# RManLuo/MAMDR

Hardware: AMD Instinct MI355X
Metric: domain-steps/sec (higher is better)
Workload: dtype f32; 1 GPU; mlp_meta_mamdr Taobao-10 bs=1024 (frozen pretrained tables); global_batch=1024, domains=10, step_definition=one MAMDR meta-epoch (DN + DR phases, all outer updates), parallelism=single GPU

## Files before the change

include/mamdr_hip.h:

```cpp
#ifndef MAMDR_HIP_H
#define MAMDR_HIP_H

#include <stddef.h>
#include <stdint.h>

#ifdef __cplusplus
extern "C" {
#endif

#define MAMDR_ABI_VERSION 19

enum {
    MAMDR_OK = 0,
    MAMDR_EINVAL = -1,
    MAMDR_ESTATE = -2,
    MAMDR_EHIP = -3,
    MAMDR_ENOTBUILT = -4
};

enum { MAMDR_TOWER_MLP = 0, MAMDR_TOWER_DEEPFM = 1, MAMDR_TOWER_STAR = 2,
       MAMDR_TOWER_WDL = 3,
       MAMDR_TOWER_PNN = 4,
       MAMDR_TOWER_NFM = 5 };
enum { MAMDR_SPLIT_TRAIN = 0, MAMDR_SPLIT_VAL = 1, MAMDR_SPLIT_TEST = 2 };
// ... 30 lines not shown
    int32_t n_item;
    int32_t n_domain;
    int32_t emb_dim;
    int32_t hidden[3];
    int32_t max_batch;
    int32_t emb_trainable;
    float dropout;
    float l2_emb;
    float l2_linear;
    float adam_beta1, adam_beta2, adam_eps;
    int32_t uncertainty_weight;
} mamdr_config;

const char* mamdr_last_error(void);
int mamdr_abi_version(void);
const char* mamdr_env_switches(void);
int mamdr_env_unknown(void);

int mamdr_create(const mamdr_config* cfg, void* stream, mamdr_ctx** out);
int mamdr_destroy(mamdr_ctx* ctx);

int64_t mamdr_param_count(const mamdr_ctx* ctx);
int64_t mamdr_meta_count(const mamdr_ctx* ctx);
int64_t mamdr_aux_count(const mamdr_ctx* ctx);
int mamdr_bind_aux(mamdr_ctx* ctx, float* d_aux);
int mamdr_param_segment(const mamdr_ctx* ctx, int seg, int64_t* offset, int64_t* count);

int mamdr_bind_state(mamdr_ctx* ctx, float* d_params, float* d_adam_m, float* d_adam_v);
int mamdr_optimizer_reset(mamdr_ctx* ctx);
int mamdr_bind_accumulator(mamdr_ctx* ctx, float* d_acc);
int64_t mamdr_optimizer_steps(const mamdr_ctx* ctx);
int mamdr_set_counters(mamdr_ctx* ctx, int64_t optimizer_steps, int64_t dropout_steps);
int mamdr_sync_tables(mamdr_ctx* ctx);
int64_t mamdr_table_flushes(const mamdr_ctx* ctx, int32_t forced_only);

int mamdr_bind_table(mamdr_ctx* ctx, int seg, const float* d_rows, int64_t n_rows);

int mamdr_bind_domain_data(mamdr_ctx* ctx, int domain, int split, const int32_t* d_uid,
                           const int32_t* d_pid, const int32_t* d_domain, const float* d_label,
                           int64_t n_rows);

int mamdr_train_steps(mamdr_ctx* ctx, int domain, const int32_t* d_perm, int64_t first_step,
                      int64_t n_steps, int32_t batch, uint32_t dropout_seed, int32_t optimizer,
                      float lr, float* d_loss_out);
int mamdr_train_steps_n(mamdr_ctx* ctx, int domain, const int32_t* d_perm, int64_t pass_rows, int64_t first_step,
                        int64_t n_steps, int32_t batch, uint32_t dropout_seed, int32_t optimizer, float lr,
                        float* d_loss_out);

int mamdr_eval_domain(mamdr_ctx* ctx, int domain, int split, int32_t batch, float* d_loss_out,
                      uint32_t* d_hist, float* d_pred_out);

int mamdr_gather_rows(mamdr_ctx* ctx, int domain, int split, const int32_t* d_perm,
                      int64_t first_row, int64_t n_rows, float* d_out);

int mamdr_interp(float* d_dst, const float* d_a, const float* d_b, float scale, int64_t n,
                 void* stream);
int mamdr_moving_average(float* d_unbiased, float* d_biased, const float* d_value, float decay, float denom,
                         int64_t n, void* stream);
int mamdr_merge(float* d_dst, const float* d_theta, const float* d_phi, int32_t mode, int64_t n,
                void* stream);
int mamdr_dr_advance(float* d_phi, float* d_w, float* d_merged, const float* d_theta, float gamma, int32_t mode,
                     int32_t assign_model, int64_t n, void* stream);
int mamdr_dr_advance_live(mamdr_ctx* ctx, float* d_phi, float* d_merged, const float* d_theta, float gamma, int32_t mode,
                          int32_t assign_model, int64_t meta_off, int64_t n);
int mamdr_sub(float* d_dst, const float* d_a, const float* d_b, int64_t n, void* stream);
int mamdr_accumulate(float* d_acc, const float* d_a, const float* d_b, const float* d_shared,
                     float divisor, int64_t n, void* stream);
int mamdr_apply_accumulated(float* d_dst, float* d_acc, float divisor, float scale, int64_t n,
                            void* stream);
int mamdr_adam_apply(float* d_p, float* d_m, float* d_v, const float* d_g, float grad_scale, float lr,
                     float beta1, float beta2, float eps, float beta1_power, float beta2_power, int64_t n,
                     void* stream);
int mamdr_copy(float* d_dst, const float* d_src, int64_t n, void* stream);
int mamdr_pcgrad_project(float* d_final, float* d_aux, const int64_t* h_offsets, const int64_t* h_rows,
                         const int32_t* h_cols, int32_t n_seg, void* stream);

int mamdr_shuffle_perm(int64_t n, int64_t buffer_size, uint64_t seed, int32_t* h_out);
int mamdr_shuffle_perms(int32_t n_passes, const int64_t* h_n, int64_t buffer_size, const uint64_t* h_seeds,
                        int32_t* h_out);

int mamdr_profile_enable(mamdr_ctx* ctx, int32_t enable);
int mamdr_pregather_passes(mamdr_ctx* ctx, int32_t n_passes, const int32_t* h_domains, const int32_t* const* h_d_perms,
                           const int64_t* h_pass_rows, int32_t batch);
int64_t mamdr_pregather_hits(const mamdr_ctx* ctx);
int64_t mamdr_pregather_launches(const mamdr_ctx* ctx);
int mamdr_step_path(const mamdr_ctx* ctx, int32_t batch);
int mamdr_set_tower_tile(mamdr_ctx* ctx, int32_t rows);
int mamdr_tower_tile(const mamdr_ctx* ctx, int32_t batch);
int64_t mamdr_dropout_steps(const mamdr_ctx* ctx);
int mamdr_profile_reset(mamdr_ctx* ctx);
int mamdr_profile_read(mamdr_ctx* ctx, int32_t kernel, double* total_ms, int64_t* launches);

enum { MAMDR_GRAPH_SHARED_BOTTOM = 0,
       MAMDR_GRAPH_MMOE = 1,
       MAMDR_GRAPH_PLE = 2,
       MAMDR_GRAPH_NFM = 3,
       MAMDR_GRAPH_PNN = 4,
       MAMDR_GRAPH_CCPM = 5,
       MAMDR_GRAPH_AUTOINT = 6,
       MAMDR_GRAPH_MLP = 7,
       MAMDR_GRAPH_WDL = 8,
       MAMDR_GRAPH_DEEPFM = 9,
       MAMDR_GRAPH_STAR = 10 };
typedef struct mamdr_graph mamdr_graph;
typedef struct mamdr_graph_config {
    int32_t abi_version;
    int32_t kind;
    int32_t n_user, n_item, n_domain, emb_dim, max_batch, emb_trainable;
    int32_t n_expert_hidden; int32_t expert_hidden[4];
    int32_t n_tower_hidden;  int32_t tower_hidden[4];
    int32_t n_gate_hidden;   int32_t gate_hidden[4];
    int32_t num_experts;
    int32_t shared_expert_num, specific_expert_num;
    float dropout, l2_emb, adam_beta1, adam_beta2, adam_eps;
    float l2_linear;
    int32_t uncertainty_weight;
    int32_t star_norm;
    int32_t star_dense;
    int32_t auxiliary_dim;
} mamdr_graph_config;
const char* mamdr_graph_last_error(void);
int mamdr_graph_create(const mamdr_graph_config* cfg, void* stream, mamdr_graph** out);
int mamdr_graph_destroy(mamdr_graph* g);
int64_t mamdr_graph_param_count(const mamdr_graph* g);
int32_t mamdr_graph_tensor_count(const mamdr_graph* g);
int mamdr_graph_tensor_info(const mamdr_graph* g, int32_t i, char* name, int32_t name_cap, int64_t* offset, int64_t* rows,
                            int64_t* cols);
int mamdr_graph_task_ranges(const mamdr_graph* g, int domain, int64_t* shared_off, int64_t* shared_count, int64_t* task_off,
                            int64_t* task_count);
int mamdr_graph_bind_state(mamdr_graph* g, float* d_params, float* d_adam_m, float* d_adam_v);
int mamdr_graph_optimizer_reset(mamdr_graph* g);
int mamdr_graph_set_adam_eps(mamdr_graph* g, float eps);
int64_t mamdr_graph_optimizer_steps(const mamdr_graph* g);
int64_t mamdr_graph_aux_count(const mamdr_graph* g);
int mamdr_graph_bind_aux(mamdr_graph* g, float* d_aux);
int64_t mamdr_graph_launch_count(void);
int64_t mamdr_graph_dropout_steps(const mamdr_graph* g);
int mamdr_graph_set_counters(mamdr_graph* g, int64_t optimizer_steps, int64_t dropout_steps);
int mamdr_graph_bind_table(mamdr_graph* g, int seg, const float* d_rows, int64_t n_rows);
int mamdr_graph_bind_domain_data(mamdr_graph* g, int domain, int split, const int32_t* d_uid, const int32_t* d_pid,
                                 const int32_t* d_domain, const float* d_label, int64_t n_rows);
int mamdr_graph_train_steps(mamdr_graph* g, int domain, const int32_t* d_perm, int64_t first_step, int64_t n_steps,
                            int32_t batch, uint32_t dropout_seed, int32_t optimizer, float lr, float* d_loss_out);
int mamdr_graph_train_steps_n(mamdr_graph* g, int domain, const int32_t* d_perm, int64_t pass_rows, int64_t first_step,
                              int64_t n_steps, int32_t batch, uint32_t dropout_seed, int32_t optimizer, float lr,
                              float* d_loss_out);
int mamdr_graph_bind_accumulator(mamdr_graph* g, float* d_acc);
int mamdr_graph_eval_domain(mamdr_graph* g, int domain, int split, int32_t batch, float* d_loss_out, uint32_t* d_hist,
                            float* d_pred_out);

#ifdef __cplusplus
}
#endif
#endif
```

mamdr_amd/_lib.py:

```python
import ctypes as C
import os

HERE = os.path.dirname(os.path.abspath(__file__))
LIB_PATH = os.environ.get("MAMDR_LIB_PATH") or os.path.join(HERE, "libmamdr_hip.so")

ABI_VERSION = 19
OK, EINVAL, ESTATE, EHIP, ENOTBUILT = 0, -1, -2, -3, -4
TOWER_MLP, TOWER_DEEPFM, TOWER_STAR, TOWER_WDL, TOWER_PNN, TOWER_NFM = 0, 1, 2, 3, 4, 5
SPLIT_TRAIN, SPLIT_VAL, SPLIT_TEST = 0, 1, 2
OPT_ADAM, OPT_SGD, OPT_ACCUMULATE = 0, 1, 2
MERGE_PLUS, MERGE_TIMES = 0, 1
(SEG_USER_EMB, SEG_ITEM_EMB, SEG_DOMAIN_EMB, SEG_W0, SEG_W1, SEG_W2, SEG_B0, SEG_B1, SEG_B2, SEG_WO,
 SEG_GB, SEG_LIN_USER, SEG_LIN_ITEM, SEG_LIN_DOMAIN) = range(14)
SEG_NAMES = ("user_emb", "item_emb", "domain_emb", "W0", "W1", "W2", "b0", "b1", "b2", "wo", "gb",
             "lin_user", "lin_item", "lin_domain",
             "Ws0", "Ws1", "Ws2", "bs0", "bs1", "bs2", "pn_gamma_shared", "pn_beta_shared", "pn_gamma_spec",
             "pn_beta_spec", "Wd0", "Wd1", "Wd2", "bd0", "bd1", "bd2",
             "log_var",
             "W0x")
KERNEL_FWD_BWD, KERNEL_WGRAD, KERNEL_UPDATE, KERNEL_EVAL, KERNEL_GATHER, KERNEL_EMB_SWEEP, KERNEL_AUX, KERNEL_FLUSH = range(8)
KERNEL_NAMES = ("k_tower<train>", "k_wgrad", "k_update", "k_tower<eval>", "k_gather", "k_emb_sweep",
                "other launches of a step (include/mamdr_hip.h: MAMDR_KERNEL_AUX)", "k_emb_flush")


class MamdrError(RuntimeError):
    def __init__(self, code, text):
        RuntimeError.__init__(self, "libmamdr_hip error %d: %s" % (code, text))
        self.code = code


class NotBuiltError(MamdrError, NotImplementedError):
    pass


class Config(C.Structure):
    _fields_ = [
        ("abi_version", C.c_int32), ("tower", C.c_int32), ("n_user", C.c_int32), ("n_item", C.c_int32),
        ("n_domain", C.c_int32), ("emb_dim", C.c_int32), ("hidden", C.c_int32 * 3), ("max_batch", C.c_int32),
        ("emb_trainable", C.c_int32), ("dropout", C.c_float), ("l2_emb", C.c_float), ("l2_linear", C.c_float),
        ("adam_beta1", C.c_float), ("adam_beta2", C.c_float), ("adam_eps", C.c_float),
        ("uncertainty_weight", C.c_int32),
    ]


GRAPH_SHARED_BOTTOM, GRAPH_MMOE, GRAPH_PLE, GRAPH_NFM, GRAPH_PNN, GRAPH_CCPM, GRAPH_AUTOINT = 0, 1, 2, 3, 4, 5, 6
GRAPH_MLP, GRAPH_WDL, GRAPH_DEEPFM = 7, 8, 9
GRAPH_STAR = 10
STAR_NORMS = {"none": 0, "pn": 1, "bn": 2}
STAR_DENSES = {"dense": 0, "star": 1}


class GraphConfig(C.Structure):
    _fields_ = [
        ("abi_version", C.c_int32), ("kind", C.c_int32), ("n_user", C.c_int32), ("n_item", C.c_int32),
        ("n_domain", C.c_int32), ("emb_dim", C.c_int32), ("max_batch", C.c_int32), ("emb_trainable", C.c_int32),
        ("n_expert_hidden", C.c_int32), ("expert_hidden", C.c_int32 * 4),
        ("n_tower_hidden", C.c_int32), ("tower_hidden", C.c_int32 * 4),
        ("n_gate_hidden", C.c_int32), ("gate_hidden", C.c_int32 * 4),
        ("num_experts", C.c_int32), ("shared_expert_num", C.c_int32), ("specific_expert_num", C.c_int32),
        ("dropout", C.c_float), ("l2_emb", C.c_float), ("adam_beta1", C.c_float), ("adam_beta2", C.c_float),
        ("adam_eps", C.c_float), ("l2_linear", C.c_float), ("uncertainty_weight", C.c_int32),
        ("star_norm", C.c_int32), ("star_dense", C.c_int32), ("auxiliary_dim", C.c_int32),
    ]


_VP, _I32, _I64, _U32, _U64, _F = C.c_void_p, C.c_int32, C.c_int64, C.c_uint32, C.c_uint64, C.c_float

SIGNATURES = {
    "mamdr_last_error": (C.c_char_p, []),
    "mamdr_abi_version": (C.c_int, []),
    "mamdr_env_switches": (C.c_char_p, []),
    "mamdr_env_unknown": (C.c_int, []),
    "mamdr_create": (C.c_int, [C.POINTER(Config), _VP, C.POINTER(_VP)]),
    "mamdr_destroy": (C.c_int, [_VP]),
    "mamdr_param_count": (_I64, [_VP]),
    "mamdr_param_segment": (C.c_int, [_VP, C.c_int, C.POINTER(_I64), C.POINTER(_I64)]),
    "mamdr_meta_count": (_I64, [_VP]),
    "mamdr_aux_count": (_I64, [_VP]),
    "mamdr_bind_aux": (C.c_int, [_VP, _VP]),
    "mamdr_bind_state": (C.c_int, [_VP, _VP, _VP, _VP]),
    "mamdr_optimizer_reset": (C.c_int, [_VP]),
    "mamdr_optimizer_steps": (_I64, [_VP]),
    "mamdr_set_counters": (C.c_int, [_VP, _I64, _I64]),
    "mamdr_table_flushes": (_I64, [_VP, _I32]),
    "mamdr_pregather_passes": (_I32, [_VP, _I32, _VP, _VP, _VP, _I32]),
    "mamdr_pregather_hits": (_I64, [_VP]),
    "mamdr_pregather_launches": (_I64, [_VP]),
    "mamdr_sync_tables": (C.c_int, [_VP]),
    "mamdr_bind_accumulator": (C.c_int, [_VP, _VP]),
    "mamdr_bind_table": (C.c_int, [_VP, C.c_int, _VP, _I64]),
    "mamdr_bind_domain_data": (C.c_int, [_VP, C.c_int, C.c_int, _VP, _VP, _VP, _VP, _I64]),
    "mamdr_train_steps": (C.c_int, [_VP, C.c_int, _VP, _I64, _I64, _I32, _U32, _I32, _F, _VP]),
    "mamdr_train_steps_n": (C.c_int, [_VP, C.c_int, _VP, _I64, _I64, _I64, _I32, _U32, _I32, _F, _VP]),
    "mamdr_eval_domain": (C.c_int, [_VP, C.c_int, C.c_int, _I32, _VP, _VP, _VP]),
    "mamdr_gather_rows": (C.c_int, [_VP, C.c_int, C.c_int, _VP, _I64, _I64, _VP]),
    "mamdr_interp": (C.c_int, [_VP, _VP, _VP, _F, _I64, _VP]),
    "mamdr_moving_average": (C.c_int, [_VP, _VP, _VP, _F, _F, _I64, _VP]),
    "mamdr_merge": (C.c_int, [_VP, _VP, _VP, _I32, _I64, _VP]),
    "mamdr_dr_advance": (C.c_int, [_VP, _VP, _VP, _VP, _F, _I32, _I32, _I64, _VP]),
    "mamdr_dr_advance_live": (C.c_int, [_VP, _VP, _VP, _VP, _F, _I32, _I32, _I64, _I64]),
    "mamdr_sub": (C.c_int, [_VP, _VP, _VP, _I64, _VP]),
    "mamdr_accumulate": (C.c_int, [_VP, _VP, _VP, _VP, _F, _I64, _VP]),
    "mamdr_apply_accumulated": (C.c_int, [_VP, _VP, _F, _F, _I64, _VP]),
    "mamdr_adam_apply": (C.c_int, [_VP, _VP, _VP, _VP, _F, _F, _F, _F, _F, _F, _F, _I64, _VP]),
    "mamdr_copy": (C.c_int, [_VP, _VP, _I64, _VP]),
    "mamdr_pcgrad_project": (C.c_int, [_VP, _VP, _VP, _VP, _VP, _I32, _VP]),
    "mamdr_shuffle_perm": (C.c_int, [_I64, _I64, _U64, _VP]),
    "mamdr_shuffle_perms": (C.c_int, [_I32, _VP, _I64, _VP, _VP]),
    "mamdr_step_path": (C.c_int, [_VP, _I32]),
    "mamdr_dropout_steps": (_I64, [_VP]),
    "mamdr_set_tower_tile": (C.c_int, [_VP, _I32]),
    "mamdr_tower_tile": (C.c_int, [_VP, _I32]),
    "mamdr_profile_enable": (C.c_int, [_VP, _I32]),
    "mamdr_profile_reset": (C.c_int, [_VP]),
    "mamdr_profile_read": (C.c_int, [_VP, _I32, C.POINTER(C.c_double), C.POINTER(_I64)]),
    "mamdr_graph_last_error": (C.c_char_p, []),
    "mamdr_graph_create": (C.c_int, [C.POINTER(GraphConfig), _VP, C.POINTER(_VP)]),
    "mamdr_graph_destroy": (C.c_int, [_VP]),
    "mamdr_graph_param_count": (_I64, [_VP]),
    "mamdr_graph_tensor_count": (_I32, [_VP]),
    "mamdr_graph_tensor_info": (C.c_int, [_VP, _I32, C.c_char_p, _I32, C.POINTER(_I64), C.POINTER(_I64), C.POINTER(_I64)]),
    "mamdr_graph_task_ranges": (C.c_int, [_VP, C.c_int, C.POINTER(_I64), C.POINTER(_I64), C.POINTER(_I64), C.POINTER(_I64)]),
    "mamdr_graph_bind_state": (C.c_int, [_VP, _VP, _VP, _VP]),
    "mamdr_graph_optimizer_reset": (C.c_int, [_VP]),
    "mamdr_graph_set_adam_eps": (C.c_int, [_VP, _F]),
    "mamdr_graph_aux_count": (_I64, [_VP]),
    "mamdr_graph_bind_aux": (C.c_int, [_VP, _VP]),
    "mamdr_graph_launch_count": (_I64, []),
    "mamdr_graph_optimizer_steps": (_I64, [_VP]),
    "mamdr_graph_dropout_steps": (_I64, [_VP]),
    "mamdr_graph_set_counters": (C.c_int, [_VP, _I64, _I64]),
    "mamdr_graph_bind_table": (C.c_int, [_VP, C.c_int, _VP, _I64]),
    "mamdr_graph_bind_domain_data": (C.c_int, [_VP, C.c_int, C.c_int, _VP, _VP, _VP, _VP, _I64]),
    "mamdr_graph_train_steps": (C.c_int, [_VP, C.c_int, _VP, _I64, _I64, _I32, _U32, _I32, _F, _VP]),
    "mamdr_graph_train_steps_n": (C.c_int, [_VP, C.c_int, _VP, _I64, _I64, _I64, _I32, _U32, _I32, _F, _VP]),
    "mamdr_graph_bind_accumulator": (C.c_int, [_VP, _VP]),
    "mamdr_graph_eval_domain": (C.c_int, [_VP, C.c_int, C.c_int, _I32, _VP, _VP, _VP]),
}

_lib = None


def load():
    global _lib
    if _lib is not None:
        return _lib
    import torch
    if not os.path.exists(LIB_PATH):
        raise ImportError("%s not found: run `python -c 'import __graft_entry__ as g; g.build()'` "
                          "(there is no CPU fallback for the MAMDR hot path)" % LIB_PATH)
    lib = C.CDLL(LIB_PATH)
    for name, (res, args) in SIGNATURES.items():
        fn = getattr(lib, name)
        fn.restype = res
        fn.argtypes = args
    if lib.mamdr_abi_version() != ABI_VERSION:
        raise ImportError("libmamdr_hip.so ABI %d != binding ABI %d" % (lib.mamdr_abi_version(), ABI_VERSION))
    lib.mamdr_env_unknown()
    _lib = lib
    return lib


def env_switches():
    rows = load().mamdr_env_switches().decode("utf-8").strip().split("\n")
    return [tuple(r.split("\t")) for r in rows]


def check(code, graph=False):
    if code != OK:
        text = (load().mamdr_graph_last_error() if graph else load().mamdr_last_error()).decode("utf-8", "replace")
# ... 5 lines not shown
```

mamdr_amd/csrc/env_registry.h:

```cpp
#pragma once

namespace mamdr {

struct EnvSwitch {
    const char* name;
    const char* reader;
    const char* effect;
};

static const EnvSwitch kEnvSwitches[] = {
    {"MAMDR_DENSE_ADAM", "lib,bench", "1: per-step dense sweep of trainable tables instead of the lazy replay (same bits)"},
    {"MAMDR_LAZY_FLUSH_EVERY", "lib", "steps between forced replays of lagging table rows (default 32)"},
    {"MAMDR_LAZY_LOG_CAP", "lib", "capacity of the alpha ring of the lazy table Adam (tests: force it to wrap)"},
    {"MAMDR_NO_TAILFUSE", "lib", "1: the table kernels as launches of their own instead of riders"},
    {"MAMDR_TOWER_TILE", "lib,bench", "rows per tower workgroup: 0 automatic, 4, 16 (initial value of mamdr_set_tower_tile)"},
    {"MAMDR_FUSED", "lib", "0: slab path everywhere; 2: k_wgrad_adam path for every batch size (default: up to 4 rows x CUs)"},
    {"MAMDR_DM_EACH", "lib", "1: k_dm_finish after every step (diagnostic; same bits)"},
    {"MAMDR_DM_CALL", "lib", "1: k_dm_finish closes every call (diagnostic; same bits)"},
    {"MAMDR_T4_NO_W1L", "lib", "1: k_tower4 without the W1 image in LDS (diagnostic)"},
    {"MAMDR_NO_W2_DIRECT", "lib", "1: k_transpose_w opens a call instead of the W2-in-place tower instance"},
    {"MAMDR_NO_PREGATHER", "lib,bench", "1: no k_pass_prep; the tower gathers its rows itself"},
    {"MAMDR_STAR_DENSE_SLICES", "lib", "1: every per-domain Star slice swept every step (diagnostic; same bits)"},
    {"MAMDR_GRAPH_NO_DEFER", "lib", "1: a pair of weight-gradient launches per layer instead of the queued flat grid"},
    {"MAMDR_GRAPH_TILE32_BELOW", "lib", "row count below which the 32 x 32 GEMM tile is used (0: 64 x 64 everywhere)"},
    {"MAMDR_GRAPH_NO_TAIL_OPT", "lib", "1: k_graph_adam as a launch of its own (same bits)"},
    {"MAMDR_LIB_PATH", "host,bench", "load this build of the library instead of mamdr_amd/libmamdr_hip.so (tools/build_variant.sh)"},
    {"MAMDR_LANES", "host", "lanes per process (overrides train.lanes)"},
    {"MAMDR_SHARE_GPU", "host", "1: every rank of run.py on device 0 over gloo (testing on a 1-GPU box)"},
    {"MAMDR_COMM_TIMEOUT", "host", "seconds: process-group timeout of run.py"},
    {"MAMDR_TAIL_SYNC", "host", "sum: tensors outside theta / phi combined by sum instead of the step-weighted mean"},
    {"MAMDR_NO_PASS_WINDOW", "host", "1: every call gathers its own pass (no k_pass_prep_multi windows)"},
    {"MAMDR_PASS_WINDOW_ROWS", "host", "row budget of a pass window"},
    {"MAMDR_PNN_ENGINE", "host", "graph: PNN on the generic-layer engine (default: step kernels)"},
    {"MAMDR_NFM_ENGINE", "host", "graph: NFM on the generic-layer engine"},
    {"MAMDR_STAR_ENGINE", "host", "graph: Star's PartitionedNorm + StarFCN form on the generic-layer engine (default: step kernels)"},
    {"MAMDR_BENCH_*", "bench", "bench.py knobs: _BATCH _ROW_SCALE _DN_MODE _NO_PREFETCH _PREP_TIMING _PREWARM_S _SHARE_GPU _COMM_TIMEOUT _SKIP_<WORKLOAD>"},
    {"MAMDR_DIAG_FLAGS", "tools", "extra -D flags of the stamp tools' diagnostic builds"},
    {"MAMDR_STAMPS_PREBUILT", "tools", "stamp tools: use an already built variant"},
    {"MAMDR_DIST_AUC_SCALE", "tools", "row scale of tools/dist_auc.py"},
    {"MAMDR_TEST_*", "tests", "test-suite knobs: _ALL_CPUS _BLAS_THREADS _NO_ORACLE_POOL _NO_PINNING _REPORT_FRAC"},
};
constexpr int kNumEnvSwitches = (int)(sizeof(kEnvSwitches) / sizeof(kEnvSwitches[0]));

}
```

mamdr_amd/csrc/fused_kernels.hip:

```cpp
#include <hip/hip_ext.h>

#include "mamdr_kernels.h"

namespace mamdr {

constexpr int FZ_THREADS = 512;
constexpr int FZ_WAVES = 8;
constexpr int FZ_RING = 32;
constexpr int FZ_SBLK = DM_PARTS;
constexpr int FZ_SC = 8;
constexpr int FZ_OUTB = 2;
constexpr int FZ_T0 = (2 * EMB / 16) * (H1 / 32);
constexpr int FZ_T1 = (H1 / 16) * (H2 / 32);
constexpr int FZ_T2 = (H2 / 16) * (H3 / 32);
constexpr int FZ_TILES = FZ_T0 + FZ_T1 + FZ_T2;

#define FZSTAMP(k) MAMDR_STAMP(MAMDR_CYCLES, a.stamps && threadIdx.x == 0, a.stamps[blockIdx.x * 8 + (k)])
#define FZREAL(k) MAMDR_STAMP(MAMDR_REALTIME, a.stamps && threadIdx.x == 0, a.stamps[blockIdx.x * 8 + (k)])

__device__ __forceinline__ void fz_store(const FusedArgs& a, int e, float p, float m, float v) {
    if (a.optimizer == 2) {
        a.m[e] = m;
        return;
    }
    if (a.optimizer == 0) {
        a.m[e] = m;
        a.v[e] = v;
    }
    a.p[e] = p;
}

__device__ __forceinline__ void fz_share(int n_slots, int w, int& s0, int& s1) {
    const int per = (n_slots + FZ_WAVES - 1) / FZ_WAVES;
    s0 = min(w * per, n_slots);
    s1 = min(s0 + per, n_slots);
}

template <bool CSUM>
__device__ __forceinline__ void fz_dense(const float* __restrict__ A, int lda, const float* __restrict__ B, int ldb,
                                         int s0, int s1, f32x4 (&acc)[2], f32x2& csum) {
    const int lane = threadIdx.x & 63, j = lane & 15, kq = lane >> 4;
    const int n = s1 - s0;
    if (n <= 0) return;
    const unsigned aoff = (unsigned)(kq * lda + j), boff = (unsigned)(kq * ldb + 2 * j);
    const float* arow = A + (size_t)(4 * s0) * lda;
    const float* brow = B + (size_t)(4 * s0) * ldb;
    const size_t astep = (size_t)4 * lda, bstep = (size_t)4 * ldb;
    const int last = n - 1;
    float ra[FZ_RING];
    f32x2 rb[FZ_RING];
#pragma unroll
    for (int u = 0; u < FZ_RING; ++u) {
        const int idx = min(u, last);
        ra[u] = (arow + idx * astep)[aoff];
        rb[u] = *reinterpret_cast<const f32x2*>(brow + idx * bstep + boff);
    }
    __builtin_amdgcn_sched_barrier(0);
    const int passes = (n + FZ_RING - 1) / FZ_RING;
    int base = 0;
    for (int pass = 0; pass + 1 < passes; ++pass, base += FZ_RING) {
#pragma unroll
        for (int u = 0; u < FZ_RING; ++u) {
            acc[0] = MAMDR_MFMA16(ra[u], rb[u][0], acc[0]);
            acc[1] = MAMDR_MFMA16(ra[u], rb[u][1], acc[1]);
            if (CSUM) csum += rb[u];
            const int idx = min(base + u + FZ_RING, last);
            ra[u] = (arow + idx * astep)[aoff];
            rb[u] = *reinterpret_cast<const f32x2*>(brow + idx * bstep + boff);
            __builtin_amdgcn_sched_barrier(0);
        }
    }
#pragma unroll
    for (int u = 0; u < FZ_RING; ++u) {
        const float keep = (base + u < n) ? 1.0f : 0.0f;
        const f32x2 b2 = rb[u] * keep;
        acc[0] = MAMDR_MFMA16(ra[u], b2[0], acc[0]);
        acc[1] = MAMDR_MFMA16(ra[u], b2[1], acc[1]);
        if (CSUM) csum += b2;
        __builtin_amdgcn_sched_barrier(0);
    }
}

template <int MT>
__device__ __forceinline__ void fz_onehot(const int32_t* __restrict__ domrow, const float* __restrict__ B, int ldb,
                                          int s0, int s1, f32x4 (&acc)[4]) {
    const int lane = threadIdx.x & 63, j = lane & 15, kq = lane >> 4;
    const int n = s1 - s0;
    if (n <= 0) return;
    const unsigned boff = (unsigned)(kq * ldb + (j & (FZ_SC - 1)));
    const int32_t* drow = domrow + 4 * s0;
    const float* brow = B + (size_t)(4 * s0) * ldb;
    const size_t bstep = (size_t)4 * ldb;
    const int last = n - 1;
    int rd[FZ_RING];
    float rb[FZ_RING];
#pragma unroll
    for (int u = 0; u < FZ_RING; ++u) {
        const int idx = min(u, last);
// ... 278 lines not shown
            rd[u] = (drow + idx * 4)[(unsigned)kq];
        }
        __builtin_amdgcn_sched_barrier(0);
        const int passes = (n + FZ_RING - 1) / FZ_RING;
        int base = 0;
        for (int pass = 0; pass + 1 < passes; ++pass, base += FZ_RING) {
#pragma unroll
            for (int u = 0; u < FZ_RING; ++u) {
                const float bv = j == 0 ? rd[u] : 0.f;
                acc[0] = MAMDR_MFMA16(ra[u][0], bv, acc[0]);
                acc[1] = MAMDR_MFMA16(ra[u][1], bv, acc[1]);
                sg += bv;
                const int idx = min(base + u + FZ_RING, last);
                ra[u] = *reinterpret_cast<const f32x2*>(arow + (size_t)idx * 4 * ACT_LD + aoff);
                rd[u] = (drow + idx * 4)[(unsigned)kq];
                __builtin_amdgcn_sched_barrier(0);
            }
        }
#pragma unroll
        for (int u = 0; u < FZ_RING; ++u) {
            const float bv = (j == 0 && base + u < n) ? rd[u] : 0.f;
            acc[0] = MAMDR_MFMA16(ra[u][0], bv, acc[0]);
            acc[1] = MAMDR_MFMA16(ra[u][1], bv, acc[1]);
            sg += bv;
            __builtin_amdgcn_sched_barrier(0);
        }
    }
    if (j == 0) {
#pragma unroll
        for (int r = 0; r < 4; ++r)
            *reinterpret_cast<f32x2*>(lds + w * 32 + 2 * (4 * kq + r)) = (f32x2){acc[0][r], acc[1][r]};
    }
    sg += __shfl_xor(sg, 16);
    sg += __shfl_xor(sg, 32);
    if (lane == 0) lds[256 + w] = sg;
    FZSTAMP(2);
    __syncthreads();
    FZSTAMP(3);
    if (tid < 32) {
        float g = lds[tid];
#pragma unroll
        for (int ww = 1; ww < FZ_WAVES; ++ww) g += lds[ww * 32 + tid];
        const int e = a.L.wo + 32 * ob + tid;
        float p = a.p[e], m = a.optimizer == 1 ? 0.f : a.m[e], v = a.optimizer == 0 ? a.v[e] : 0.f;
        opt_step(a, g, p, m, v);
        fz_store(a, e, p, m, v);
    } else if (tid == 64 && ob == 0) {
        float g = lds[256];
#pragma unroll
        for (int ww = 1; ww < FZ_WAVES; ++ww) g += lds[256 + ww];
        const int e = a.L.gb;
        float p = a.p[e], m = a.optimizer == 1 ? 0.f : a.m[e], v = a.optimizer == 0 ? a.v[e] : 0.f;
        opt_step(a, g, p, m, v);
        fz_store(a, e, p, m, v);
    }
    FZSTAMP(4);
}

__device__ __forceinline__ void fz_loss_body(const FusedArgs& a, float* lds) {
    const int tid = threadIdx.x;
    float ss = 0.f, ls = 0.f;
    for (int e = tid; e < a.n_domain * EMB; e += FZ_THREADS) ss = fmaf(a.p[e], a.p[e], ss);
    for (int e = tid; e < a.n_loss_tiles; e += FZ_THREADS) ls += a.loss_part[e];
    for (int o = 32; o > 0; o >>= 1) {
        ss += __shfl_xor(ss, o);
        ls += __shfl_xor(ls, o);
    }
    if ((tid & 63) == 0) {
        lds[tid >> 6] = ss;
        lds[8 + (tid >> 6)] = ls;
    }
    __syncthreads();
    if (tid == 0) {
        float sst = 0.f, lst = 0.f;
        for (int ww = 0; ww < FZ_WAVES; ++ww) {
            sst += lds[ww];
            lst += lds[8 + ww];
        }
        const float reg = a.l2_emb * a.frozen_sumsq[0] + a.l2_emb * a.frozen_sumsq[1] + a.l2_emb * sst;
        a.loss_out[0] = lst / (float)a.rows + reg;
    }
}

__global__ __launch_bounds__(FZ_THREADS) void k_wgrad_adam(const FusedArgs a) {
    extern __shared__ __attribute__((aligned(16))) float lds[];
    const int b = (int)blockIdx.x;
    FZSTAMP(0);
    FZREAL(5);
    if (b < FZ_SBLK) fz_s_body(a, b, lds);
    else if (b < FZ_SBLK + FZ_TILES) fz_tile_body(a, b - FZ_SBLK, lds);
    else if (b < FZ_SBLK + FZ_TILES + FZ_OUTB) fz_out_body(a, b - FZ_SBLK - FZ_TILES, lds);
    else fz_loss_body(a, lds);
    FZREAL(6);
}

void launch_wgrad_adam(const FusedArgs& a, hipStream_t s) {
    const int grid = FZ_SBLK + FZ_TILES + FZ_OUTB + (a.loss_out ? 1 : 0);
    const size_t lds = (size_t)fz_lds_floats(a.n_domain) * sizeof(float);
    if (lds > 65536) {
        static const bool big_lds_set = hipFuncSetAttribute(reinterpret_cast<const void*>(k_wgrad_adam),
                                                            hipFuncAttributeMaxDynamicSharedMemorySize,
                                                            (int)(fz_lds_floats(64) * sizeof(float))) == hipSuccess;
        (void)big_lds_set;
    }
    MAMDR_LAUNCH(k_wgrad_adam, dim3(grid), dim3(FZ_THREADS), lds, s, a);
}

__global__ __launch_bounds__(256) void k_dm_finish(const DmStep q, float* live_p, float* live_m, float* live_v) {
    const int i = blockIdx.x * 256 + threadIdx.x;
    if (i >= q.n_domain * (EMB / 4)) return;
    const int d = i / (EMB / 4), c4 = i - d * (EMB / 4);
    f32x4 p, m, v;
    dm_step4(q, d, c4, p, m, v);
    const size_t row = (size_t)d * EMB + 4 * c4;
    if (q.optimizer != 2) *reinterpret_cast<f32x4*>(live_p + row) = p;
    if (q.optimizer != 1) *reinterpret_cast<f32x4*>(live_m + row) = m;
    if (q.optimizer == 0) *reinterpret_cast<f32x4*>(live_v + row) = v;
}

void launch_dm_finish(const DmStep& q, float* live_p, float* live_m, float* live_v, hipStream_t s) {
    MAMDR_LAUNCH(k_dm_finish, dim3((q.n_domain * (EMB / 4) + 255) / 256), dim3(256), 0, s, q, live_p, live_m, live_v);
}

template <typename P>
__device__ __forceinline__ void pass_prep_row(const P& a, const float* user_tab, const float* item_tab, int n_user, int n_item,
                                              int n_domain, int64_t pos0, float* xpre, int32_t* pdom, float* plabel, int64_t i) {
    const int lane = threadIdx.x & 63;
    if (i >= a.n) {
        if (i < a.n + 16) {
            *reinterpret_cast<f32x4*>(xpre + (size_t)i * (2 * EMB) + 4 * lane) = (f32x4){0.f, 0.f, 0.f, 0.f};
            if (lane == 0) {
                pdom[i] = a.pad_dom;
                plabel[i] = 0.f;
            }
        }
        return;
    }
    int64_t src = a.perm ? (int64_t)a.perm[pos0 + i] : pos0 + i;
    src = src < 0 ? 0 : (src >= a.n_rows_split ? a.n_rows_split - 1 : src);
    int u = a.uid[src], it = a.pid[src];
    u = u < 0 ? 0 : (u >= n_user ? n_user - 1 : u);
    it = it < 0 ? 0 : (it >= n_item ? n_item - 1 : it);
    const float* row = lane < 32 ? user_tab + (size_t)u * EMB + 4 * lane : item_tab + (size_t)it * EMB + 4 * (lane - 32);
    const f32x4 v = *reinterpret_cast<const f32x4*>(row);
    __builtin_nontemporal_store(v, reinterpret_cast<f32x4*>(xpre + (size_t)i * (2 * EMB) + 4 * lane));
    if (lane == 0) {
        int d = a.dom[src];
        pdom[i] = d < 0 ? 0 : (d >= n_domain ? n_domain - 1 : d);
        plabel[i] = a.label[src];
    }
}
__global__ __launch_bounds__(256) void k_pass_prep(const PassPrepArgs a) {
    if ((int)blockIdx.x >= a.n_prep_wgs) {
        transpose_w_elem(a.tw_dense, a.tw_L, a.tw_wT, ((int)blockIdx.x - a.n_prep_wgs) * 256 + (int)threadIdx.x);
        return;
    }
    pass_prep_row(a, a.user_tab, a.item_tab, a.n_user, a.n_item, a.n_domain, a.pos0, a.xpre, a.pdom, a.plabel,
                  (int64_t)blockIdx.x * 4 + (threadIdx.x >> 6));
}
__global__ __launch_bounds__(256) void k_pass_prep_multi(const PassPrepMultiArgs a) {
    int k = 0;
    while (k + 1 < a.n_pass && (int)blockIdx.x >= a.wg_end[k]) ++k;
    const int wg0 = k ? a.wg_end[k - 1] : 0;
    const PassPrepMultiArgs::Pass& p = a.p[k];
    pass_prep_row(p, a.user_tab, a.item_tab, a.n_user, a.n_item, a.n_domain, (int64_t)0, a.xpre + (size_t)p.out_off * (2 * EMB),
                  a.pdom + p.out_off, a.plabel + p.out_off, (int64_t)((int)blockIdx.x - wg0) * 4 + (threadIdx.x >> 6));
}
void launch_pass_prep_multi(const PassPrepMultiArgs& a, hipStream_t s) {
    if (a.n_pass <= 0) return;
    MAMDR_LAUNCH(k_pass_prep_multi, dim3((unsigned)a.wg_end[a.n_pass - 1]), dim3(256), 0, s, a);
}
void launch_pass_prep(const PassPrepArgs& a0, hipStream_t s) {
    if (a0.n <= 0) return;
    PassPrepArgs a = a0;
    a.n_prep_wgs = (int)((a.n + 16 + 3) / 4);
    MAMDR_LAUNCH(k_pass_prep, dim3((unsigned)(a.n_prep_wgs + (a.tw_wT ? TRANSPOSE_WGS : 0))), dim3(256), 0, s, a);
}

}
```

mamdr_amd/csrc/mamdr_api.hip:

```cpp
#include <hip/hip_runtime.h>

#include <cmath>
#include <cstdarg>
#include <cstdio>
#include <cstdlib>
#include <cstring>
#include <new>
#include <string>
#include <utility>
#include <vector>

#include "../../include/mamdr_hip.h"
#include "mamdr_kernels.h"
#include "env_registry.h"

using namespace mamdr;

namespace mamdr {
thread_local hipEvent_t g_prof_stop = nullptr;
}

namespace {

thread_local char g_err[512] = "";
// ... 4 lines not shown
    vsnprintf(g_err, sizeof(g_err), fmt, ap);
    va_end(ap);
    return code;
}

#define HIP_TRY(expr)                                                                          \
    do {                                                                                       \
        hipError_t e_ = (expr);                                                                \
        if (e_ != hipSuccess) return fail(MAMDR_EHIP, "%s: %s", #expr, hipGetErrorString(e_)); \
    } while (0)

struct SplitData {
    const int32_t* uid = nullptr;
    const int32_t* pid = nullptr;
    const int32_t* dom = nullptr;
    const float* label = nullptr;
    int64_t n = 0;
    bool bound = false;
};

struct EventPair {
    hipEvent_t a, b;
    bool own_a = true;
};

}

struct mamdr_ctx {
    mamdr_config cfg;
    hipStream_t stream = nullptr;
    DenseLayout L;
    int64_t table_floats = 0;
    bool deepfm = false;
    bool nfm = false;
    bool pnn = false;
    float* ipbuf = nullptr;
    bool star = false;
    StarLayout SL;
    StarAuxLayout AL;
    int64_t n_meta = 0;
    float* aux = nullptr;
    float* eff = nullptr;
    float* pn = nullptr;
    float* star_part = nullptr;
    float* star_sums = nullptr;
    float* star_dmpart = nullptr;
    int64_t lin_user_off = 0;
    int64_t lin_item_off = 0;
    int64_t n_params = 0;
    float* params = nullptr;
    float* adam_m = nullptr;
    float* adam_v = nullptr;
    float* accum = nullptr;
    const float* user_tab = nullptr;
    const float* item_tab = nullptr;
    std::vector<SplitData> data;
    int64_t adam_t = 0;
    float b1p = 1.0f, b2p = 1.0f;
    uint32_t global_step = 0;
    int rows_pad_max = 0;
    float* acts = nullptr;
    float* dz = nullptr;
    float* dlogit = nullptr;
    float* w0dom_copy = nullptr;
    float* dm_copy = nullptr;
    bool lin_w0dom = false;
    float* wT = nullptr;
    bool fused = false;
    float* star_alpha = nullptr;
    int star_dense_slices = 0;
    int t4_no_w1l = 0;
    int fused_max_batch = 1024;
    int tower4_max_rows = 2048;
    float* pdm = nullptr;
    float* xpre = nullptr;
    int32_t* pdom = nullptr;
    float* plabel = nullptr;
    int64_t pre_cap = 0;
    struct PgEntry { int domain; const int32_t* perm; int64_t n, off; int batch; };
    std::vector<PgEntry> pg;
    size_t pg_pos = 0;
    int64_t pg_hits = 0;
    int64_t pg_launches = 0;
    bool use_pre = true;
    float* dmsnap[2] = {nullptr, nullptr};
    int dm_cur = 0;
    DmStep dm_pending{};
    bool dm_finish_call = false;
    bool wT_valid = false;
    bool w1t_unread = false;
    bool w2_direct_ok = true;
    bool dm_finish_each = false;
    int tower_tile = 0;
    float* dxe = nullptr;
    int32_t* urow = nullptr;
    int32_t* irow = nullptr;
    int32_t* map_u = nullptr;
    int32_t* map_i = nullptr;
    float* gbuf_u = nullptr;
    float* gbuf_i = nullptr;
    int32_t* hasdup_u = nullptr;
    int32_t* hasdup_i = nullptr;
    bool lazy = false;
    bool tables_dirty = false;
    int32_t* last_u = nullptr;
    int32_t* last_i = nullptr;
    float* alpha_log = nullptr;
    int log_cap = 1 << 16;
    int flush_every = 32;
    int64_t flush_t = 0;
    int64_t n_flush = 0;
    int64_t n_flush_forced = 0;
    float* fmq = nullptr;
    float* glin_u = nullptr;
    float* glin_i = nullptr;
    int32_t* domrow = nullptr;
    float* loss_part = nullptr;
    float* eval_part = nullptr;
    int64_t eval_part_cap = 0;
    float* slabs = nullptr;
    bool tail_fuse = true;
    int32_t* urow_alt = nullptr;
    int32_t* irow_alt = nullptr;
    int32_t* map_u_alt = nullptr;
    int32_t* map_i_alt = nullptr;
    bool rows_ready = false;
    bool catchup_ready = false;
    int slab_ld = 0;
    int s2_off = 0;
    TileDesc* tiles = nullptr;
    int n_tiles = 0;
    float* thresholds = nullptr;
    float* frozen_sumsq = nullptr;
    float* sumsq_partials = nullptr;
#ifdef MAMDR_STAMPS
    unsigned long long* stamps = nullptr;
#endif
    bool profile = false;
    std::vector<hipEvent_t> ev_pool;
    void ev_pool_push(hipEvent_t e) { ev_pool.push_back(e); }
    hipEvent_t prev_b = nullptr;
    bool chain_ok = false;
    std::vector<EventPair> ev[MAMDR_KERNEL_COUNT];
};

namespace {

std::vector<TileDesc> build_tiles(const DenseLayout& L, int n_domain, bool deepfm, int s2_off, bool lin_w0dom, bool star,
                                  bool pnn = false, bool nfm = false) {
    std::vector<TileDesc> t;
    struct G { int a_off, M, b_off, N, dst; };
    const G gemms[3] = {{0, XDIM, 0, H1, L.w0}, {XDIM, H1, H1, H2, L.w1}, {XDIM + H1, H2, H1 + H2, H3, L.w2}};
    for (const G& g : gemms)
        for (int m0 = (nfm && g.dst == L.w0) ? 2 * EMB : 0; m0 < ((lin_w0dom && g.dst == L.w0) ? 2 * EMB : g.M); m0 += 64)
            for (int n0 = 0; n0 < g.N; n0 += 64)
                t.push_back(TileDesc{0, g.a_off + m0, 0, g.b_off + n0, g.dst + m0 * g.N + n0, g.N, 64, 64, 1});
    const int boff[3] = {L.b0, L.b1, L.b2}, bn[3] = {H1, H2, H3}, zoff[3] = {0, H1, H1 + H2};
    for (int l = 0; l < 3; ++l)
        for (int n0 = 0; n0 < bn[l]; n0 += 32) t.push_back(TileDesc{1, 0, 0, zoff[l] + n0, boff[l] + n0, 0, 1, 32});
    for (int m0 = 0; m0 < H3; m0 += 32) t.push_back(TileDesc{0, XDIM + H1 + H2 + m0, 1, 0, L.wo + m0, 1, 32, 1});
    t.push_back(TileDesc{1, 0, 1, 0, L.gb, 0, 1, 1});
    for (int m0 = 0; m0 < (star ? 0 : n_domain); m0 += 32)
        for (int n0 = 0; n0 < H1; n0 += 32) {
            const int mv = n_domain - m0 < 32 ? n_domain - m0 : 32;
            t.push_back(TileDesc{2, m0, 0, n0, L.alloc + m0 * H1 + n0, H1, mv, 32});
        }
// ... 169 lines not shown
    }
    c->tables_dirty = false;
    c->flush_t = c->adam_t;
    c->n_flush += 1;
}

static void fill_rows_args(const mamdr_ctx* c, const SplitData& d, const int32_t* d_perm, int64_t row_base, int rows,
                           int rows_pad, float alpha, int64_t t, bool alt, EmbRowsArgs& ra) {
    memset(&ra, 0, sizeof(ra));
    ra.uid = d.uid;
    ra.pid = d.pid;
    ra.perm = d_perm;
    ra.row_base = row_base;
    ra.n_rows_split = d.n;
    ra.rows = rows;
    ra.rows_pad = rows_pad;
    ra.n_user = c->cfg.n_user;
    ra.n_item = c->cfg.n_item;
    ra.urow = alt ? c->urow_alt : c->urow;
    ra.irow = alt ? c->irow_alt : c->irow;
    ra.map_u = alt ? c->map_u_alt : c->map_u;
    ra.map_i = alt ? c->map_i_alt : c->map_i;
    ra.alpha_log = c->alpha_log;
    ra.log_idx = (int)(t & (c->log_cap - 1));
    ra.alpha = alpha;
}

static void emb_pre_step(mamdr_ctx* c, const SplitData& d, const int32_t* d_perm, int64_t row_base, int rows,
                         int rows_pad, float alpha, float omb1, float omb2) {
    if (c->adam_t - c->flush_t >= c->log_cap - 2 || c->adam_t - c->flush_t > c->flush_every) {
        c->adam_t -= 1;
        if (c->tables_dirty) c->n_flush_forced += 1;
        sync_tables(c);
        c->adam_t += 1;
    }
    if (!c->rows_ready) {
        EmbRowsArgs ra;
        fill_rows_args(c, d, d_perm, row_base, rows, rows_pad, alpha, c->adam_t, false, ra);
        Prof p(c, MAMDR_KERNEL_AUX);
        launch_emb_rows(ra, c->stream);
    }
    c->rows_ready = false;
    if (!c->catchup_ready) {
        EmbStepArgs ea;
        fill_emb_args(c, MAMDR_OPT_ADAM, alpha, omb1, omb2, table_two_l2(c), rows, c->star ? XDIM : 2 * EMB, ea);
        Prof p(c, MAMDR_KERNEL_AUX);
        launch_emb_catchup(ea, c->stream);
    }
    c->catchup_ready = false;
    c->tables_dirty = true;
}

static void emb_post_step(mamdr_ctx* c, int32_t optimizer, float alpha, float omb1, float omb2, int rows) {
    EmbStepArgs ea;
    fill_emb_args(c, optimizer, alpha, omb1, omb2, table_two_l2(c), rows, c->star ? XDIM : 2 * EMB, ea);
    if (c->lazy && optimizer == MAMDR_OPT_ADAM) {
        ea.flags_done = 1;
        ea.apply_now = 1;
        {
            Prof p(c, MAMDR_KERNEL_EMB_SWEEP);
            launch_emb_reduce(ea, c->stream);
        }
        if (c->deepfm) {
            Prof p(c, MAMDR_KERNEL_AUX);
            launch_lin_sweep(ea, c->stream);
        }
        return;
    }
    launch_emb_reduce(ea, c->stream);
    prof_break(c);
    {
        Prof p(c, MAMDR_KERNEL_EMB_SWEEP);
        launch_emb_sweep(ea, c->stream);
    }
    if (c->deepfm) {
        Prof p(c, MAMDR_KERNEL_AUX);
        launch_lin_sweep(ea, c->stream);
    }
}

static int64_t pad_rows(int64_t rows) { return (rows + TILE_ROWS - 1) / TILE_ROWS * TILE_ROWS; }
static int rows_at(int64_t pass_rows, int64_t row_base, int batch) { return (int)std::min<int64_t>(batch, pass_rows - row_base); }
static bool takes_fused_path(const mamdr_ctx* c, int64_t batch) { return c->fused && pad_rows(batch) <= c->fused_max_batch; }
static bool takes_tower4(const mamdr_ctx* c, int64_t rows_pad) {
    return !c->star && c->tower_tile != 16 && (c->tower_tile == 4 || rows_pad <= c->tower4_max_rows);
}
static bool w1t_unread_now(const mamdr_ctx* c) {
    if (!c->fused || c->tower_tile == 16) return false;
    const int64_t max4 = c->tower_tile == 4 ? c->rows_pad_max : std::min<int64_t>(c->tower4_max_rows, c->rows_pad_max);
    return tower4_never_streams(max4, c->t4_no_w1l);
}
static int wgrad_groups(int rows_pad, int* rpg) {
    int r = rows_pad <= 512 ? 256 : (rows_pad <= 1024 ? 128 : (rows_pad <= 4096 ? 256 : 512));
    int groups = (rows_pad + r - 1) / r;
    if (groups > WGRAD_MAX_GROUPS) {
        r = ((rows_pad + WGRAD_MAX_GROUPS - 1) / WGRAD_MAX_GROUPS + 7) / 8 * 8;
        groups = (rows_pad + r - 1) / r;
    }
    *rpg = r;
    return groups;
}
static float adam_alpha(float lr, float b1p, float b2p) { return lr * sqrtf(1.0f - b2p) / (1.0f - b1p); }
static float advance_step(mamdr_ctx* c, int32_t optimizer, float lr) {
    if (optimizer != MAMDR_OPT_ADAM) return lr;
    c->adam_t += 1;
    c->b1p = c->b1p * c->cfg.adam_beta1;
    c->b2p = c->b2p * c->cfg.adam_beta2;
    return adam_alpha(lr, c->b1p, c->b2p);
}

enum class StepPath { star, fused, slab };
struct CallPlan {
    const SplitData* d;
    int domain;
    const int32_t* perm;
    int64_t pass_rows, first_step, n_steps;
    int batch;
    int32_t optimizer;
    float lr, omb1, omb2;
    float* loss_out;
    uint32_t seed, drop_thresh;
    float keep_scale;
    int use_dropout;
    StepPath path = StepPath::slab;
    bool tail = false;
    bool pre = false;
    bool pre_cached = false;
    int64_t pre_pos0 = 0, pre_n = 0, pre_base = 0;
    bool need_wT = false;
    bool build_wT = false;
    bool w2_direct = false;
    bool star_lazy = false;
};

static void plan_call(mamdr_ctx* c, CallPlan& P) {
    P.path = c->star ? StepPath::star : (takes_fused_path(c, P.batch) ? StepPath::fused : StepPath::slab);
    const bool fused = P.path == StepPath::fused;
    const bool accumulate = P.optimizer == MAMDR_OPT_ACCUMULATE;
    P.tail = c->tail_fuse && c->cfg.emb_trainable && c->lazy && P.optimizer == MAMDR_OPT_ADAM && !c->profile && !P.loss_out;
    const int first_rows = rows_at(P.pass_rows, P.first_step * P.batch, P.batch);
    P.need_wT = takes_tower4(c, pad_rows(rows_at(P.pass_rows, (P.first_step + P.n_steps - 1) * P.batch, P.batch)));
    P.pre_pos0 = P.first_step * P.batch;
    P.pre_n = std::min<int64_t>((P.first_step + P.n_steps) * P.batch, P.pass_rows) - P.pre_pos0;
    P.pre = fused && c->use_pre && P.pre_n > 0;
    P.build_wT = P.need_wT && !c->wT_valid;
    if (P.build_wT && P.pre && c->w2_direct_ok && !accumulate && !c->t4_no_w1l && c->tower_tile != 16 && tower4_w1l_ready() &&
        tower4_takes_w1l(first_rows, c->t4_no_w1l)) {
        P.build_wT = false;
        P.w2_direct = true;
    }
    if (P.build_wT && !accumulate && !fused && !c->star && !takes_tower4(c, pad_rows(first_rows)) && P.n_steps > 1)
        P.build_wT = false;
    if (P.pre) {
        for (size_t k = c->pg_pos; k < c->pg.size(); ++k) {
            const mamdr_ctx::PgEntry& e = c->pg[k];
            if (e.domain == P.domain && e.perm == P.perm && e.n == P.pass_rows && e.batch == P.batch) {
                c->pg_pos = k;
                P.pre_base = e.off + P.pre_pos0;
                P.pre_cached = true;
                c->pg_hits += 1;
                break;
            }
        }
        if (!P.pre_cached) c->pg.clear();
    }
    P.star_lazy = c->star && P.optimizer == MAMDR_OPT_ADAM && P.n_steps >= 2 && !P.loss_out && !c->star_dense_slices &&
                  c->cfg.n_domain > 1;
}

static void fill_next_step(const mamdr_ctx* c, const CallPlan& P, int64_t row_base, EmbRowsArgs& nr, EmbStepArgs& nea) {
    const int rows = rows_at(P.pass_rows, row_base, P.batch);
    const float alpha = adam_alpha(P.lr, c->b1p * c->cfg.adam_beta1, c->b2p * c->cfg.adam_beta2);
    fill_rows_args(c, *P.d, P.perm, row_base, rows, (int)pad_rows(rows), alpha, c->adam_t + 1, true, nr);
    fill_emb_args(c, MAMDR_OPT_ADAM, alpha, P.omb1, P.omb2, table_two_l2(c), rows, c->star ? XDIM : 2 * EMB, nea);
    nea.t_now = (int)c->adam_t + 1;
    nea.t[0].brow = c->urow_alt;
    nea.t[0].map = c->map_u_alt;
    nea.t[1].brow = c->irow_alt;
    nea.t[1].map = c->map_i_alt;
}

static void take_next_rows(mamdr_ctx* c) {
    std::swap(c->urow, c->urow_alt);
    std::swap(c->irow, c->irow_alt);
    std::swap(c->map_u, c->map_u_alt);
    std::swap(c->map_i, c->map_i_alt);
    c->rows_ready = true;
    c->catchup_ready = true;
    c->tables_dirty = true;
}

static int star_step(mamdr_ctx* c, const CallPlan& P, int64_t s, float alpha) {
    const SplitData& d = *P.d;
    const int domain = P.domain;
    const int32_t optimizer = P.optimizer;
    const float omb1 = P.omb1, omb2 = P.omb2;
    float* const loss_out = P.loss_out ? P.loss_out + s : nullptr;
    const int64_t row_base = (P.first_step + s) * P.batch;
    const int rows = rows_at(P.pass_rows, row_base, P.batch);
    const int rows_pad = (int)pad_rows(rows);
    const int chunks = (rows + STAR_CHUNK - 1) / STAR_CHUNK;
    const int lazy_idx = (int)(s & (STAR_ALPHA_CAP - 1));
    const bool next = P.tail && s + 1 < P.n_steps;
    EmbRowsArgs nr;
    EmbStepArgs nea;
    if (next) fill_next_step(c, P, row_base + P.batch, nr, nea);
    float* blk = c->params + c->table_floats;
    TowerArgs ta;
    fill_tower_common(c, d, ta);
    ta.perm = P.perm;
    ta.row_base = row_base;
    ta.rows = rows;
    ta.batch = rows;
    if (c->cfg.emb_trainable && c->lazy && optimizer == MAMDR_OPT_ADAM)
        emb_pre_step(c, d, P.perm, row_base, rows, rows_pad, alpha, omb1, omb2);
    StarPrepArgs pa;
    memset(&pa, 0, sizeof(pa));
    pa.blk = blk;
    pa.SL = c->SL;
    pa.L = c->L;
    pa.n_domain = c->cfg.n_domain;
    pa.d = domain;
    pa.eff = c->eff;
    pa.pn = c->pn;
    pa.part = c->star_part;
    pa.n_chunks = chunks;
    pa.rows = rows;
    pa.aux = c->aux;
    pa.AL = c->AL;
    pa.train = 1;
    pa.skip_eff = P.star_lazy && s > 0 ? 1 : 0;
    {
        Prof p(c, MAMDR_KERNEL_AUX);
        launch_star_stats(ta, c->star_part, c->aux + c->AL.steps + domain, c->stream);
        launch_star_prep(pa, c->stream);
    }

    ta.dense = c->eff;
    ta.pn_aff = c->pn;
    ta.pn_part = c->star_part;
    ta.use_dropout = 0;
    ta.keep_scale = 1.0f;
    ta.acts = c->acts;
    ta.dz = c->dz;
    ta.dlogit = c->dlogit;
    ta.domrow = c->domrow;
    ta.dxe = c->dxe;
// ... 101 lines not shown
    ua.opt.eps = c->cfg.adam_eps;
    ua.opt.two_l2 = 0.f;
    if (P.star_lazy) {
        ua.only_live = 1;
        ua.alpha_log = c->star_alpha;
        ua.log_idx = lazy_idx;
        if (s + 1 < P.n_steps) ua.eff_out = c->eff;
    }
    {
        Prof p(c, MAMDR_KERNEL_UPDATE);
        ua.dm_elsewhere = no_apply ? 1 : 0;
        if (next) launch_star_update_catchup(ua, nea, no_apply ? &ba : nullptr, c->stream);
        else launch_star_update(ua, c->stream);
    }
    if (next) take_next_rows(c);
    if (c->cfg.emb_trainable && !P.tail) emb_post_step(c, optimizer, alpha, omb1, omb2, rows);
    c->global_step += 1;
    if (P.star_lazy && (lazy_idx + 1 == STAR_ALPHA_CAP || s + 1 == P.n_steps)) {
        StarCatchArgs ca;
        memset(&ca, 0, sizeof(ca));
        ca.p = c->params + c->table_floats;
        ca.m = c->adam_m + c->table_floats;
        ca.v = c->adam_v + c->table_floats;
        ca.SL = c->SL;
        ca.n_domain = c->cfg.n_domain;
        ca.d_live = domain;
        ca.alpha_log = c->star_alpha;
        ca.first_idx = 0;
        ca.n_steps = lazy_idx + 1;
        ca.log_mask = STAR_ALPHA_CAP - 1;
        ca.omb1 = omb1;
        ca.omb2 = omb2;
        ca.eps = c->cfg.adam_eps;
        Prof p(c, MAMDR_KERNEL_AUX);
        launch_star_catchup(ca, c->stream);
    }
    return MAMDR_OK;
}

static void fill_step_tower(const mamdr_ctx* c, const CallPlan& P, int64_t row_base, int rows, TowerArgs& ta) {
    fill_tower_common(c, *P.d, ta);
    ta.perm = P.perm;
    ta.row_base = row_base;
    ta.rows = rows;
    ta.batch = rows;
    ta.seed = P.seed;
    ta.step = c->global_step;
    ta.drop_thresh = P.drop_thresh;
    ta.keep_scale = P.keep_scale;
    ta.use_dropout = P.use_dropout;
    ta.acts = c->acts;
    ta.dz = c->dz;
    ta.dlogit = c->dlogit;
    ta.domrow = c->domrow;
    ta.dxe = c->dxe;
    ta.dx_ld = 2 * EMB;
    ta.urow = c->urow;
    ta.irow = c->irow;
    ta.map_u = c->map_u;
    ta.map_i = c->map_i;
    ta.loss_part = c->loss_part;
    ta.fmq = c->fmq;
    if (c->L.lv_count > 0) ta.uw_off = c->L.lv + P.domain;
#ifdef MAMDR_STAMPS
    ta.stamps = c->stamps ? c->stamps + (c->global_step & 1) * 16384 : nullptr;
#endif
    ta.wT = c->wT;
    ta.no_w1l = c->t4_no_w1l;
}

static int run_step_tower(mamdr_ctx* c, const TowerArgs& ta, bool use4, int64_t s) {
    if ((c->pnn || c->nfm) && !use4)
        return fail(MAMDR_ENOTBUILT, "pnn / nfm tower: a training step of %d rows needs the four-row tower (MAMDR_TOWER_TILE=16?)", ta.rows);
    Prof p(c, MAMDR_KERNEL_FWD_BWD);
#ifdef MAMDR_TOWER_TWICE
    if (use4) (void)launch_tower4_train(ta, c->stream);
#endif
    const int t4e = use4 ? launch_tower4_train(ta, c->stream) : (launch_tower_train(ta, c->stream), 0);
    if (t4e == T4_E_W2D_LDS) return fail(MAMDR_EHIP, "k_tower4<W2D> was refused its LDS limit (hipFuncSetAttribute)");
    if (t4e) return fail(MAMDR_ESTATE, "w2_direct without the W1-image instance of k_tower4 (step %lld of the call)", (long long)s);
    return MAMDR_OK;
}

static int fused_step(mamdr_ctx* c, const CallPlan& P, int64_t s, float alpha) {
    const int32_t optimizer = P.optimizer;
    const int64_t row_base = (P.first_step + s) * P.batch;
    const int rows = rows_at(P.pass_rows, row_base, P.batch);
    const int rows_pad = (int)pad_rows(rows);
    const bool use4 = takes_tower4(c, rows_pad);
    DmStep& dm_pending = c->dm_pending;
    float* const dense_m = (optimizer == MAMDR_OPT_ACCUMULATE ? c->accum : c->adam_m) + c->table_floats;
    TowerArgs ta;
    fill_step_tower(c, P, row_base, rows, ta);
    c->dm_cur ^= 1;
    ta.dms = dm_pending;
    ta.dm_hint = P.domain;
    if (P.pre) {
        const int64_t at = P.pre_base + row_base - P.pre_pos0;
        ta.xpre = c->xpre + (size_t)at * 2 * EMB;
        ta.pdom = c->pdom + at;
        ta.plabel = c->plabel + at;
    }
    ta.dm_live_p = c->params + c->table_floats + c->L.dm;
    ta.dm_live_m = dense_m + c->L.dm;
    ta.dm_live_v = c->adam_v + c->table_floats + c->L.dm;
    ta.dm_snap_out = c->dmsnap[c->dm_cur];
    ta.w2_direct = (P.w2_direct && s == 0) ? 1 : 0;
    if (int rc = run_step_tower(c, ta, use4, s)) return rc;
    FusedArgs fa;
    memset(&fa, 0, sizeof(fa));
    fa.acts = c->acts;
    fa.dz = c->dz;
    fa.dlogit = c->dlogit;
    fa.domrow = c->domrow;
    fa.xa = ta.xpre ? ta.xpre : c->acts;
    fa.xa_ld = ta.xpre ? 2 * EMB : ACT_LD;
    fa.rows_pad = rows_pad;
    fa.rows = rows;
    fa.p = c->params + c->table_floats;
    fa.m = dense_m;
    fa.v = c->adam_v + c->table_floats;
    fa.L = c->L;
    fa.n_domain = c->cfg.n_domain;
    fa.dm_snap = c->dmsnap[c->dm_cur];
    fa.pdm = c->pdm;
    fa.wT = (P.need_wT && optimizer != MAMDR_OPT_ACCUMULATE) ? c->wT : nullptr;
    fa.w1t_unread = c->w1t_unread ? 1 : 0;
    fa.optimizer = optimizer;
    fa.alpha = alpha;
    fa.omb1 = P.omb1;
    fa.omb2 = P.omb2;
    fa.eps = c->cfg.adam_eps;
    fa.two_l2 = 2.0f * c->cfg.l2_emb;
    fa.loss_part = c->loss_part;
    fa.n_loss_tiles = use4 ? rows_pad / 4 : rows_pad / TILE_ROWS;
    fa.frozen_sumsq = c->frozen_sumsq;
    fa.l2_emb = c->cfg.l2_emb;
    fa.loss_out = P.loss_out ? P.loss_out + s : nullptr;
#ifdef MAMDR_STAMPS
    fa.stamps = c->stamps ? c->stamps + 65536 + (c->global_step & 1) * 4096 : nullptr;
#endif
    {
        Prof p(c, MAMDR_KERNEL_WGRAD);
        launch_wgrad_adam(fa, c->stream);
    }
    dm_pending.snap = c->dmsnap[c->dm_cur];
    dm_pending.pdm = c->pdm;
    dm_pending.n_part = DM_PARTS;
    dm_pending.n_domain = c->cfg.n_domain;
    dm_pending.optimizer = optimizer;
    dm_pending.alpha = alpha;
    dm_pending.omb1 = P.omb1;
    dm_pending.omb2 = P.omb2;
    dm_pending.eps = c->cfg.adam_eps;
    dm_pending.two_l2 = 2.0f * c->cfg.l2_emb;
    if (c->dm_finish_each || (s + 1 == P.n_steps && (optimizer != MAMDR_OPT_ADAM || c->dm_finish_call))) finish_dm(c);
    c->global_step += 1;
    return MAMDR_OK;
}

static int slab_step(mamdr_ctx* c, const CallPlan& P, int64_t s, float alpha) {
    const SplitData& d = *P.d;
    const int32_t optimizer = P.optimizer;
    const float omb1 = P.omb1, omb2 = P.omb2;
    const int64_t row_base = (P.first_step + s) * P.batch;
    const int rows = rows_at(P.pass_rows, row_base, P.batch);
    const int rows_pad = (int)pad_rows(rows);
    const bool use4 = takes_tower4(c, rows_pad);
    if (c->cfg.emb_trainable && c->lazy && optimizer == MAMDR_OPT_ADAM)
        emb_pre_step(c, d, P.perm, row_base, rows, rows_pad, alpha, omb1, omb2);
    TowerArgs ta;
    fill_step_tower(c, P, row_base, rows, ta);
    if (int rc = run_step_tower(c, ta, use4, s)) return rc;

    if (c->cfg.emb_trainable && P.loss_out) {
        prof_break(c);
        launch_sumsq(c->params, (int64_t)c->cfg.n_user * EMB, c->sumsq_partials, c->frozen_sumsq + 0, c->stream);
        launch_sumsq(c->params + (size_t)c->cfg.n_user * EMB, (int64_t)c->cfg.n_item * EMB, c->sumsq_partials,
                     c->frozen_sumsq + 1, c->stream);
        if (c->deepfm) {
            launch_sumsq(c->params + c->lin_user_off, c->cfg.n_user, c->sumsq_partials, c->frozen_sumsq + 2, c->stream);
            launch_sumsq(c->params + c->lin_item_off, c->cfg.n_item, c->sumsq_partials, c->frozen_sumsq + 3, c->stream);
        }
    }
    WgradArgs wa;
    memset(&wa, 0, sizeof(wa));
    wa.acts = c->acts;
    wa.dz = c->dz;
    wa.dlogit = c->dlogit;
    wa.domrow = c->domrow;
    wa.fmq = c->fmq;
    wa.ipbuf = c->ipbuf;
    wa.ld_off = c->L.ld;
    wa.ld_count = c->L.ld_count;
    wa.l2_lin = c->cfg.l2_linear;
    wa.lv_off = c->L.lv;
    wa.lv_count = c->L.lv_count;
    wa.uw_d = P.domain;
    wa.tiles = c->tiles;
    wa.n_tiles = c->n_tiles;
    wa.rows_pad = rows_pad;
    int rpg = 0;
    const int groups = wgrad_groups(rows_pad, &rpg);
    wa.n_groups = groups;
    wa.rows_per_group = rpg;
    wa.slabs = c->slabs;
    wa.slab_ld = c->slab_ld;
    wa.w0dom = c->params + c->table_floats + c->L.w0 + (size_t)(2 * EMB) * H1;
    wa.w0dom_copy = c->w0dom_copy;
    wa.dm_copy = c->lin_w0dom ? c->dm_copy : nullptr;
    wa.loss_part = c->loss_part;
    wa.n_loss_tiles = use4 ? rows_pad / 4 : rows_pad / TILE_ROWS;
    wa.rows = rows;
    wa.dense = c->params + c->table_floats;
    wa.dm_count = c->cfg.n_domain * EMB;
    wa.l2_emb = c->cfg.l2_emb;
    wa.frozen_sumsq = c->frozen_sumsq;
    wa.loss_out = P.loss_out ? P.loss_out + s : nullptr;
#ifdef MAMDR_STAMPS
    wa.stamps = c->stamps ? c->stamps + 65536 : nullptr;
#endif
    EmbStepArgs tea, nea;
    EmbRowsArgs nr;
    const bool next = P.tail && s + 1 < P.n_steps;
// ... 168 lines not shown
    c->rows_pad_max = cfg->max_batch;
    if (const char* tt = getenv("MAMDR_TOWER_TILE")) c->tower_tile = atoi(tt);
    c->slab_ld = c->L.alloc + cfg->n_domain * H1;
    if (c->deepfm || c->pnn) {
        c->s2_off = c->slab_ld;
        c->slab_ld += cfg->n_domain * EMB;
    }

    const size_t rp = (size_t)c->rows_pad_max;
    c->lin_w0dom = (c->star || cfg->n_domain <= 64) && !c->nfm;
    std::vector<TileDesc> tiles = build_tiles(c->L, cfg->n_domain, c->deepfm, c->s2_off, c->lin_w0dom, c->star, c->pnn, c->nfm);
    c->n_tiles = (int)tiles.size();
    float thr[500];
    thr[0] = (float)(0.0 - 1e-7);
    for (int i = 0; i < 498; ++i) thr[i + 1] = (float)((double)(i + 1) * 1.0 / (double)(500 - 1));
    thr[499] = (float)(1.0 + 1e-7);

#define ALLOC(ptr, bytes)                                                        \
    do {                                                                         \
        hipError_t e_ = hipMalloc((void**)&(ptr), (bytes));                      \
        if (e_ != hipSuccess) {                                                  \
            mamdr_destroy(c);                                                    \
            return fail(MAMDR_EHIP, "hipMalloc(%zu): %s", (size_t)(bytes), hipGetErrorString(e_)); \
        }                                                                        \
    } while (0)
    ALLOC(c->acts, rp * ACT_LD * sizeof(float));
    ALLOC(c->dz, rp * DZ_LD * sizeof(float));
    ALLOC(c->dlogit, rp * sizeof(float));
    ALLOC(c->w0dom_copy, (size_t)EMB * H1 * sizeof(float));
    ALLOC(c->dm_copy, (size_t)cfg->n_domain * EMB * sizeof(float));
    if (c->star) {
        const size_t chunks = (rp + STAR_CHUNK - 1) / STAR_CHUNK;
        ALLOC(c->eff, (size_t)c->L.alloc * sizeof(float));
        ALLOC(c->pn, (size_t)PN_WS_FLOATS * sizeof(float));
        ALLOC(c->star_alpha, (size_t)STAR_ALPHA_CAP * sizeof(float));
        if (const char* sd = getenv("MAMDR_STAR_DENSE_SLICES")) c->star_dense_slices = atoi(sd) != 0;
        ALLOC(c->star_part, chunks * 2 * XDIM * sizeof(double));
        ALLOC(c->star_sums, (4 * XDIM + EMB) * sizeof(float));
        ALLOC(c->star_dmpart, chunks * EMB * sizeof(float));
    }
    if (cfg->emb_trainable || c->star) {
        ALLOC(c->dxe, rp * (c->star ? XDIM : 2 * EMB) * sizeof(float));
        ALLOC(c->urow, rp * sizeof(int32_t));
        ALLOC(c->irow, rp * sizeof(int32_t));
    }
    if (cfg->emb_trainable) {
        ALLOC(c->map_u, (size_t)cfg->n_user * sizeof(int32_t));
        ALLOC(c->map_i, (size_t)cfg->n_item * sizeof(int32_t));
        ALLOC(c->urow_alt, rp * sizeof(int32_t));
        ALLOC(c->irow_alt, rp * sizeof(int32_t));
        ALLOC(c->map_u_alt, (size_t)cfg->n_user * sizeof(int32_t));
        ALLOC(c->map_i_alt, (size_t)cfg->n_item * sizeof(int32_t));
        ALLOC(c->gbuf_u, rp * EMB * sizeof(float));
        ALLOC(c->gbuf_i, rp * EMB * sizeof(float));
        ALLOC(c->hasdup_u, rp * sizeof(int32_t));
        ALLOC(c->hasdup_i, rp * sizeof(int32_t));
        const char* dense_env = getenv("MAMDR_DENSE_ADAM");
        c->lazy = !(dense_env && atoi(dense_env) != 0);
        if (const char* fe = getenv("MAMDR_LAZY_FLUSH_EVERY")) c->flush_every = atoi(fe) > 0 ? atoi(fe) : c->flush_every;
        if (const char* cap_env = getenv("MAMDR_LAZY_LOG_CAP")) {
            const int cap = atoi(cap_env);
            if (cap >= 4 && (cap & (cap - 1)) == 0) c->log_cap = cap;
        }
        ALLOC(c->last_u, (size_t)cfg->n_user * sizeof(int32_t));
        ALLOC(c->last_i, (size_t)cfg->n_item * sizeof(int32_t));
        ALLOC(c->alpha_log, (size_t)c->log_cap * sizeof(float));
        if (c->deepfm) {
            ALLOC(c->glin_u, rp * sizeof(float));
            ALLOC(c->glin_i, rp * sizeof(float));
        }
    }
    if (c->deepfm || c->pnn) ALLOC(c->fmq, rp * EMB * sizeof(float));
    if (c->pnn) ALLOC(c->ipbuf, rp * 4 * sizeof(float));
    ALLOC(c->domrow, rp * sizeof(int32_t));
    ALLOC(c->loss_part, (rp / 4) * sizeof(float));
    ALLOC(c->wT, (size_t)WT_FLOATS * sizeof(float));
    {
        if (const char* nw = getenv("MAMDR_T4_NO_W1L")) c->t4_no_w1l = atoi(nw) != 0;
        {
            int dev = 0, n_cu = 0;
            if (hipGetDevice(&dev) != hipSuccess || hipDeviceGetAttribute(&n_cu, hipDeviceAttributeMultiprocessorCount, dev) != hipSuccess ||
                n_cu <= 0)
                n_cu = 256;
            const int one_round = std::min(2048, std::max(256, 4 * n_cu));
            c->fused_max_batch = one_round;
            if (cfg->tower == MAMDR_TOWER_MLP && !cfg->emb_trainable) c->tower4_max_rows = one_round;
        }
        const char* fe = getenv("MAMDR_FUSED");
        c->fused = cfg->tower == MAMDR_TOWER_MLP && !cfg->emb_trainable && !cfg->uncertainty_weight && c->lin_w0dom &&
                   cfg->n_domain <= 64 && !(fe && atoi(fe) == 0);
        if (c->fused && fe && atoi(fe) == 2) c->fused_max_batch = 1 << 30;
        if (c->fused) {
            ALLOC(c->pdm, (size_t)DM_PARTS * cfg->n_domain * EMB * sizeof(float));
            ALLOC(c->dmsnap[0], (size_t)3 * cfg->n_domain * EMB * sizeof(float));
            ALLOC(c->dmsnap[1], (size_t)3 * cfg->n_domain * EMB * sizeof(float));
            if (const char* de = getenv("MAMDR_DM_EACH")) c->dm_finish_each = atoi(de) != 0;
            if (const char* de = getenv("MAMDR_DM_CALL")) c->dm_finish_call = atoi(de) != 0;
            if (const char* de = getenv("MAMDR_NO_W2_DIRECT")) c->w2_direct_ok = atoi(de) == 0;
            if (const char* pe = getenv("MAMDR_NO_PREGATHER")) c->use_pre = atoi(pe) == 0;
        }
        c->w1t_unread = w1t_unread_now(c);
    }
    if (const char* ev = getenv("MAMDR_NO_TAILFUSE")) c->tail_fuse = atoi(ev) == 0;
    ALLOC(c->slabs, (size_t)WGRAD_MAX_GROUPS * c->slab_ld * sizeof(float));
    ALLOC(c->tiles, tiles.size() * sizeof(TileDesc));
    ALLOC(c->thresholds, sizeof(thr));
    ALLOC(c->frozen_sumsq, 4 * sizeof(float));
    ALLOC(c->sumsq_partials, 1024 * sizeof(float));
#undef ALLOC
    hipError_t e = hipMemsetAsync(c->slabs, 0, (size_t)WGRAD_MAX_GROUPS * c->slab_ld * sizeof(float), c->stream);
    if (e == hipSuccess) e = hipMemsetAsync(c->frozen_sumsq, 0, 4 * sizeof(float), c->stream);
    if (cfg->emb_trainable) {
        if (e == hipSuccess) e = hipMemsetAsync(c->hasdup_u, 0, rp * sizeof(int32_t), c->stream);
        if (e == hipSuccess) e = hipMemsetAsync(c->hasdup_i, 0, rp * sizeof(int32_t), c->stream);
        if (e == hipSuccess) e = hipMemsetAsync(c->last_u, 0, (size_t)cfg->n_user * sizeof(int32_t), c->stream);
        if (e == hipSuccess) e = hipMemsetAsync(c->last_i, 0, (size_t)cfg->n_item * sizeof(int32_t), c->stream);
        if (e == hipSuccess) e = hipMemsetAsync(c->alpha_log, 0, (size_t)c->log_cap * sizeof(float), c->stream);
        launch_emb_map_init(c->map_u, cfg->n_user, c->stream);
        launch_emb_map_init(c->map_i, cfg->n_item, c->stream);
        launch_emb_map_init(c->map_u_alt, cfg->n_user, c->stream);
        launch_emb_map_init(c->map_i_alt, cfg->n_item, c->stream);
    }
    if (e == hipSuccess) e = hipMemcpyAsync(c->tiles, tiles.data(), tiles.size() * sizeof(TileDesc), hipMemcpyHostToDevice, c->stream);
    if (e == hipSuccess) e = hipMemcpyAsync(c->thresholds, thr, sizeof(thr), hipMemcpyHostToDevice, c->stream);
    if (e == hipSuccess) e = hipStreamSynchronize(c->stream);
    if (e != hipSuccess) {
        mamdr_destroy(c);
        return fail(MAMDR_EHIP, "workspace initialisation: %s", hipGetErrorString(e));
    }
    *out = c;
    return MAMDR_OK;
}

int mamdr_destroy(mamdr_ctx* c) {
    if (!c) return MAMDR_OK;
    for (int k = 0; k < MAMDR_KERNEL_COUNT; ++k)
        for (EventPair& p : c->ev[k]) {
            if (p.own_a) (void)hipEventDestroy(p.a);
            (void)hipEventDestroy(p.b);
        }
    for (hipEvent_t e : c->ev_pool) (void)hipEventDestroy(e);
    void* ptrs[] = {c->urow_alt, c->irow_alt, c->map_u_alt, c->map_i_alt, c->acts, c->dz, c->dlogit, c->w0dom_copy, c->dm_copy, c->wT, c->dxe, c->urow, c->irow, c->map_u, c->map_i, c->gbuf_u, c->gbuf_i, c->hasdup_u, c->hasdup_i, c->last_u, c->last_i, c->alpha_log, c->star_alpha, c->pdm, c->dmsnap[0], c->dmsnap[1], c->xpre, c->pdom, c->plabel, c->fmq, c->ipbuf, c->glin_u, c->glin_i, c->eff, c->pn, c->star_part, c->star_sums, c->star_dmpart, c->domrow, c->loss_part, c->eval_part, c->slabs,
                    c->tiles, c->thresholds, c->frozen_sumsq, c->sumsq_partials};
    for (void* p : ptrs)
        if (p) (void)hipFree(p);
    delete c;
    return MAMDR_OK;
}

int64_t mamdr_param_count(const mamdr_ctx* c) { return c ? c->n_params : 0; }
int64_t mamdr_meta_count(const mamdr_ctx* c) { return c ? c->n_meta : 0; }
int64_t mamdr_aux_count(const mamdr_ctx* c) { return (c && c->star) ? c->AL.count : 0; }

int mamdr_bind_aux(mamdr_ctx* c, float* d_aux) {
    if (check_ctx(c)) return MAMDR_EINVAL;
    if (!c->star) return fail(MAMDR_ESTATE, "this tower has no auxiliary state");
    if (!d_aux || ((uintptr_t)d_aux & 15)) return fail(MAMDR_EINVAL, "aux pointer null or not 16-byte aligned");
    c->aux = d_aux;
    return MAMDR_OK;
}

int mamdr_param_segment(const mamdr_ctx* c, int seg, int64_t* offset, int64_t* count) {
    if (check_ctx(c)) return MAMDR_EINVAL;
    if (!offset || !count) return fail(MAMDR_EINVAL, "null argument");
    const DenseLayout& L = c->L;
    const int64_t base = c->table_floats;
    int64_t off = 0, cnt = 0;
    if (c->star) {
        const StarLayout& S = c->SL;
        const int64_t D = c->cfg.n_domain;
        const bool tr = c->cfg.emb_trainable != 0;
        if (seg >= MAMDR_SEG_STAR_WS0 && seg <= MAMDR_SEG_STAR_WS2) {
            off = base + S.ws[seg - MAMDR_SEG_STAR_WS0]; cnt = StarLayout::ksize(seg - MAMDR_SEG_STAR_WS0);
        } else if (seg >= MAMDR_SEG_STAR_BS0 && seg <= MAMDR_SEG_STAR_BS2) {
            off = base + S.bs[seg - MAMDR_SEG_STAR_BS0]; cnt = StarLayout::bsize(seg - MAMDR_SEG_STAR_BS0);
        } else if (seg >= MAMDR_SEG_STAR_WD0 && seg <= MAMDR_SEG_STAR_WD2) {
            off = base + S.wd[seg - MAMDR_SEG_STAR_WD0]; cnt = D * StarLayout::ksize(seg - MAMDR_SEG_STAR_WD0);
        } else if (seg >= MAMDR_SEG_STAR_BD0 && seg <= MAMDR_SEG_STAR_BD2) {
            off = base + S.bd[seg - MAMDR_SEG_STAR_BD0]; cnt = D * StarLayout::bsize(seg - MAMDR_SEG_STAR_BD0);
        } else {
            switch (seg) {
                case MAMDR_SEG_USER_EMB: off = 0; cnt = tr ? (int64_t)c->cfg.n_user * EMB : 0; break;
                case MAMDR_SEG_ITEM_EMB: off = tr ? (int64_t)c->cfg.n_user * EMB : 0; cnt = tr ? (int64_t)c->cfg.n_item * EMB : 0; break;
                case MAMDR_SEG_DOMAIN_EMB: off = base + S.dm; cnt = D * EMB; break;
                case MAMDR_SEG_PN_GAMMA_SHARED: off = base + S.pgs; cnt = XDIM; break;
                case MAMDR_SEG_PN_BETA_SHARED: off = base + S.pbs; cnt = XDIM; break;
                case MAMDR_SEG_PN_GAMMA_SPEC: off = base + S.pgd; cnt = D * XDIM; break;
                case MAMDR_SEG_PN_BETA_SPEC: off = base + S.pbd; cnt = D * XDIM; break;
                case MAMDR_SEG_WO: off = base + S.wo; cnt = H3; break;
                case MAMDR_SEG_GB: off = base + S.gb; cnt = 1; break;
                default:
                    if (seg < 0 || seg >= MAMDR_SEG_COUNT) return fail(MAMDR_EINVAL, "unknown segment %d", seg);
                    off = 0; cnt = 0;
            }
        }
        *offset = off;
        *count = cnt;
        return MAMDR_OK;
    }
    if (seg >= MAMDR_SEG_STAR_WS0 && seg <= MAMDR_SEG_STAR_BD2) {
        *offset = 0;
        *count = 0;
        return MAMDR_OK;
    }
    switch (seg) {
        case MAMDR_SEG_USER_EMB: off = 0; cnt = c->cfg.emb_trainable ? (int64_t)c->cfg.n_user * EMB : 0; break;
        case MAMDR_SEG_ITEM_EMB:
            off = c->cfg.emb_trainable ? (int64_t)c->cfg.n_user * EMB : 0;
            cnt = c->cfg.emb_trainable ? (int64_t)c->cfg.n_item * EMB : 0;
            break;
        case MAMDR_SEG_DOMAIN_EMB: off = base + L.dm; cnt = (int64_t)c->cfg.n_domain * EMB; break;
        case MAMDR_SEG_W0:
            off = base + L.w0 + (c->nfm ? 2 * EMB * H1 : 0);
            cnt = c->nfm ? EMB * H1 : XDIM * H1;
            break;
        case MAMDR_SEG_W1: off = base + L.w1; cnt = H1 * H2; break;
        case MAMDR_SEG_W2: off = base + L.w2; cnt = H2 * H3; break;
        case MAMDR_SEG_B0: off = base + L.b0; cnt = H1; break;
        case MAMDR_SEG_B1: off = base + L.b1; cnt = H2; break;
        case MAMDR_SEG_B2: off = base + L.b2; cnt = H3; break;
        case MAMDR_SEG_WO: off = base + L.wo; cnt = H3; break;
        case MAMDR_SEG_GB: off = base + L.gb; cnt = 1; break;
        case MAMDR_SEG_LIN_USER:
            off = c->lin_user_off;
            cnt = (c->deepfm && c->cfg.emb_trainable) ? c->cfg.n_user : 0;
// ... 9 lines not shown
    }
    *offset = off;
    *count = cnt;
    return MAMDR_OK;
}

int mamdr_bind_state(mamdr_ctx* c, float* d_params, float* d_adam_m, float* d_adam_v) {
    if (check_ctx(c)) return MAMDR_EINVAL;
    if (!d_params || !d_adam_m || !d_adam_v) return fail(MAMDR_EINVAL, "null state pointer");
    if (((uintptr_t)d_params | (uintptr_t)d_adam_m | (uintptr_t)d_adam_v) & 15)
        return fail(MAMDR_EINVAL, "state pointers must be 16-byte aligned");
    if (c->params) sync_tables(c);
    c->params = d_params;
    c->adam_m = d_adam_m;
    c->adam_v = d_adam_v;
    return MAMDR_OK;
}

int mamdr_optimizer_reset(mamdr_ctx* c) {
    if (check_ctx(c)) return MAMDR_EINVAL;
    if (!c->adam_m) return fail(MAMDR_ESTATE, "mamdr_bind_state has not been called");
    sync_tables(c);
    if (c->last_u) {
        HIP_TRY(hipMemsetAsync(c->last_u, 0, (size_t)c->cfg.n_user * sizeof(int32_t), c->stream));
        HIP_TRY(hipMemsetAsync(c->last_i, 0, (size_t)c->cfg.n_item * sizeof(int32_t), c->stream));
    }
    c->flush_t = 0;
    HIP_TRY(hipMemsetAsync(c->adam_m, 0, (size_t)c->n_params * sizeof(float), c->stream));
    HIP_TRY(hipMemsetAsync(c->adam_v, 0, (size_t)c->n_params * sizeof(float), c->stream));
    c->adam_t = 0;
    c->b1p = 1.0f;
    c->b2p = 1.0f;
    return MAMDR_OK;
}

int64_t mamdr_optimizer_steps(const mamdr_ctx* c) { return c ? c->adam_t : 0; }

int mamdr_set_counters(mamdr_ctx* c, int64_t optimizer_steps, int64_t dropout_steps) {
    if (check_ctx(c)) return MAMDR_EINVAL;
    if (optimizer_steps < 0 || optimizer_steps > (int64_t)0x7ffffff0 || dropout_steps < 0 || dropout_steps > (int64_t)0xffffffffLL)
        return fail(MAMDR_EINVAL, "mamdr_set_counters(%lld, %lld): out of range", (long long)optimizer_steps, (long long)dropout_steps);
    if (!c->adam_m) return fail(MAMDR_ESTATE, "mamdr_bind_state has not been called");
    sync_tables(c);
    if (c->last_u) {
        HIP_TRY(hipMemsetD32Async(reinterpret_cast<hipDeviceptr_t>(c->last_u), (int)optimizer_steps, (size_t)c->cfg.n_user, c->stream));
        HIP_TRY(hipMemsetD32Async(reinterpret_cast<hipDeviceptr_t>(c->last_i), (int)optimizer_steps, (size_t)c->cfg.n_item, c->stream));
    }
    c->flush_t = optimizer_steps;
    c->adam_t = optimizer_steps;
    float b1 = 1.0f, b2 = 1.0f;
    for (int64_t t = 0; t < optimizer_steps; ++t) {
        const float n1 = b1 * c->cfg.adam_beta1, n2 = b2 * c->cfg.adam_beta2;
        if (n1 == b1 && n2 == b2) break;
        b1 = n1;
        b2 = n2;
    }
    c->b1p = b1;
    c->b2p = b2;
    c->global_step = (uint32_t)dropout_steps;
    return MAMDR_OK;
}
int64_t mamdr_table_flushes(const mamdr_ctx* c, int32_t forced_only) {
    return !c ? 0 : forced_only ? c->n_flush_forced : c->n_flush;
}

int mamdr_sync_tables(mamdr_ctx* c) {
    if (check_ctx(c)) return MAMDR_EINVAL;
    sync_tables(c);
    HIP_TRY(hipGetLastError());
    return MAMDR_OK;
}

int mamdr_bind_accumulator(mamdr_ctx* c, float* d_acc) {
    if (check_ctx(c)) return MAMDR_EINVAL;
    if (!d_acc || ((uintptr_t)d_acc & 15)) return fail(MAMDR_EINVAL, "accumulator pointer null or not 16-byte aligned");
    c->accum = d_acc;
    return MAMDR_OK;
}

int mamdr_bind_table(mamdr_ctx* c, int seg, const float* d_rows, int64_t n_rows) {
    if (check_ctx(c)) return MAMDR_EINVAL;
    if (c->cfg.emb_trainable) return fail(MAMDR_ESTATE, "tables are trainable: they live in the flat vector");
    if (!d_rows || ((uintptr_t)d_rows & 15)) return fail(MAMDR_EINVAL, "table pointer null or not 16-byte aligned");
    c->pg.clear();
    if (seg == MAMDR_SEG_USER_EMB) {
        if (n_rows != c->cfg.n_user) return fail(MAMDR_EINVAL, "user table has %lld rows, config says %d", (long long)n_rows, c->cfg.n_user);
        c->user_tab = d_rows;
        launch_sumsq(d_rows, n_rows * EMB, c->sumsq_partials, c->frozen_sumsq + 0, c->stream);
    } else if (seg == MAMDR_SEG_ITEM_EMB) {
        if (n_rows != c->cfg.n_item) return fail(MAMDR_EINVAL, "item table has %lld rows, config says %d", (long long)n_rows, c->cfg.n_item);
        c->item_tab = d_rows;
        launch_sumsq(d_rows, n_rows * EMB, c->sumsq_partials, c->frozen_sumsq + 1, c->stream);
    } else {
        return fail(MAMDR_EINVAL, "segment %d is not a bindable table", seg);
    }
    HIP_TRY(hipGetLastError());
    return MAMDR_OK;
}

int mamdr_bind_domain_data(mamdr_ctx* c, int domain, int split, const int32_t* d_uid, const int32_t* d_pid,
                           const int32_t* d_domain, const float* d_label, int64_t n_rows) {
    if (check_ctx(c)) return MAMDR_EINVAL;
    SplitData* d = split_of(c, domain, split);
    if (!d) return fail(MAMDR_EINVAL, "domain %d / split %d out of range", domain, split);
    if (n_rows < 0 || n_rows > 0x7fffffff) return fail(MAMDR_EINVAL, "n_rows out of range");
    if (n_rows > 0 && (!d_uid || !d_pid || !d_domain || !d_label)) return fail(MAMDR_EINVAL, "null column pointer");
    d->bound = true;
    d->uid = d_uid;
    d->pid = d_pid;
    d->dom = d_domain;
    d->label = d_label;
    d->n = n_rows;
    c->pg.clear();
    const int64_t tiles = (n_rows + TILE_ROWS - 1) / TILE_ROWS;
    if (tiles > c->eval_part_cap) {
        HIP_TRY(hipStreamSynchronize(c->stream));
        if (c->eval_part) HIP_TRY(hipFree(c->eval_part));
        c->eval_part = nullptr;
        HIP_TRY(hipMalloc((void**)&c->eval_part, (size_t)tiles * sizeof(float)));
        c->eval_part_cap = tiles;
    }
    return MAMDR_OK;
}

static int grow_pass_buffer(mamdr_ctx* c, int64_t rows) {
    if (rows <= c->pre_cap) return MAMDR_OK;
    const int64_t cap = rows + rows / 4 + 1024;
    c->pg.clear();
    if (c->xpre) { (void)hipFree(c->xpre); (void)hipFree(c->pdom); (void)hipFree(c->plabel); }
    c->xpre = nullptr; c->pdom = nullptr; c->plabel = nullptr; c->pre_cap = 0;
    HIP_TRY(hipMalloc((void**)&c->xpre, (size_t)cap * 2 * EMB * sizeof(float)));
    HIP_TRY(hipMalloc((void**)&c->pdom, (size_t)cap * sizeof(int32_t)));
    HIP_TRY(hipMalloc((void**)&c->plabel, (size_t)cap * sizeof(float)));
    c->pre_cap = cap;
    return MAMDR_OK;
}

int64_t mamdr_pregather_hits(const mamdr_ctx* c) { return c ? c->pg_hits : 0; }
int64_t mamdr_pregather_launches(const mamdr_ctx* c) { return c ? c->pg_launches : 0; }

int mamdr_pregather_passes(mamdr_ctx* c, int32_t n_passes, const int32_t* h_domains, const int32_t* const* h_d_perms,
                           const int64_t* h_pass_rows, int32_t batch) {
    if (check_ctx(c)) return MAMDR_EINVAL;
    if (ready(c)) return MAMDR_ESTATE;
    if (n_passes < 0 || (n_passes > 0 && !h_domains)) return fail(MAMDR_EINVAL, "pregather: bad pass list");
    c->pg.clear();
    c->pg_pos = 0;
    if (n_passes == 0 || batch <= 0 || batch > c->cfg.max_batch || !c->use_pre || !takes_fused_path(c, batch))
        return MAMDR_OK;
    if (n_passes > PREP_MAX_PASSES) n_passes = PREP_MAX_PASSES;
    PassPrepMultiArgs a;
    memset(&a, 0, sizeof(a));
    int64_t off = 0;
    int wgs = 0;
    for (int k = 0; k < n_passes; ++k) {
        SplitData* d = split_of(c, h_domains[k], MAMDR_SPLIT_TRAIN);
        if (!d || !d->bound) return fail(MAMDR_ESTATE, "pregather: train split of domain %d is not bound", h_domains[k]);
        int64_t n = h_pass_rows ? h_pass_rows[k] : -1;
        if (n < 0) n = d->n;
        if (n > d->n) return fail(MAMDR_EINVAL, "pregather: pass of %lld rows exceeds the %lld rows of domain %d", (long long)n,
                                  (long long)d->n, h_domains[k]);
        PassPrepMultiArgs::Pass& p = a.p[k];
        p.uid = d->uid;
        p.pid = d->pid;
        p.dom = d->dom;
        p.label = d->label;
        p.perm = h_d_perms ? h_d_perms[k] : nullptr;
        p.n = n;
        p.n_rows_split = d->n;
        p.out_off = off;
        p.pad_dom = h_domains[k];
        const int64_t w = n > 0 ? (n + 16 + 3) / 4 : 0;
        wgs += (int)w;
        a.wg_end[k] = wgs;
        c->pg.push_back(mamdr_ctx::PgEntry{h_domains[k], p.perm, n, off, batch});
        off += 4 * w;
    }
    a.n_pass = n_passes;
    if (wgs == 0) return MAMDR_OK;
    {
        std::vector<mamdr_ctx::PgEntry> keep = c->pg;
        if (int rc = grow_pass_buffer(c, off)) return rc;
        c->pg = keep;
    }
    a.user_tab = c->user_tab;
    a.item_tab = c->item_tab;
    a.n_user = c->cfg.n_user;
    a.n_item = c->cfg.n_item;
    a.n_domain = c->cfg.n_domain;
    a.xpre = c->xpre;
    a.pdom = c->pdom;
    a.plabel = c->plabel;
    prof_break(c);
    {
        Prof p(c, MAMDR_KERNEL_AUX);
        launch_pass_prep_multi(a, c->stream);
        c->pg_launches++;
    }
    HIP_TRY(hipGetLastError());
    return MAMDR_OK;
}

int mamdr_train_steps(mamdr_ctx* c, int domain, const int32_t* d_perm, int64_t first_step, int64_t n_steps,
                      int32_t batch, uint32_t dropout_seed, int32_t optimizer, float lr, float* d_loss_out) {
    return mamdr_train_steps_n(c, domain, d_perm, -1, first_step, n_steps, batch, dropout_seed, optimizer, lr, d_loss_out);
}

int mamdr_train_steps_n(mamdr_ctx* c, int domain, const int32_t* d_perm, int64_t pass_rows, int64_t first_step,
                        int64_t n_steps, int32_t batch, uint32_t dropout_seed, int32_t optimizer, float lr,
                        float* d_loss_out) {
    if (check_ctx(c)) return MAMDR_EINVAL;
    if (ready(c)) return MAMDR_ESTATE;
    SplitData* d = split_of(c, domain, MAMDR_SPLIT_TRAIN);
    if (!d || !d->bound) return fail(MAMDR_ESTATE, "train split of domain %d is not bound", domain);
    if (batch <= 0 || batch > c->cfg.max_batch) return fail(MAMDR_EINVAL, "batch %d outside (0, max_batch=%d]", batch, c->cfg.max_batch);
    if (optimizer != MAMDR_OPT_ADAM && optimizer != MAMDR_OPT_SGD && optimizer != MAMDR_OPT_ACCUMULATE)
        return fail(MAMDR_EINVAL, "unknown optimizer %d", optimizer);
    if (optimizer == MAMDR_OPT_ACCUMULATE && !c->accum)
        return fail(MAMDR_ESTATE, "MAMDR_OPT_ACCUMULATE needs mamdr_bind_accumulator first");
    if (first_step < 0 || n_steps < 0) return fail(MAMDR_EINVAL, "negative step range");
    if (pass_rows < 0) pass_rows = d->n;
    if (pass_rows > d->n) return fail(MAMDR_EINVAL, "pass of %lld rows exceeds the %lld rows of domain %d",
                                      (long long)pass_rows, (long long)d->n, domain);
    const int64_t pass_steps = (pass_rows + batch - 1) / batch;
    if (first_step + n_steps > pass_steps)
        return fail(MAMDR_EINVAL, "steps [%lld,%lld) exceed the %lld batches of domain %d", (long long)first_step,
                    (long long)(first_step + n_steps), (long long)pass_steps, domain);
    if (n_steps == 0) return MAMDR_OK;

    const float rate = c->cfg.dropout;
    double thr = (double)rate * 4294967296.0;
    const uint32_t drop_thresh = thr >= 4294967295.0 ? 0xFFFFFFFFu : (uint32_t)(int64_t)thr;
    const float keep_scale = (float)(1.0 / (1.0 - (double)rate));
    const float omb1 = 1.0f - c->cfg.adam_beta1, omb2 = 1.0f - c->cfg.adam_beta2;
    const int use_dropout = (rate > 0.f && optimizer != MAMDR_OPT_ACCUMULATE) ? 1 : 0;
    CallPlan P{d, domain, d_perm, pass_rows, first_step, n_steps, batch, optimizer, lr, omb1, omb2, d_loss_out,
               dropout_seed, drop_thresh, keep_scale, use_dropout};
    if (optimizer != MAMDR_OPT_ADAM) sync_tables(c);
    plan_call(c, P);

    c->rows_ready = false;
    c->catchup_ready = false;
    prof_break(c);
    if (!(P.path == StepPath::fused && optimizer == MAMDR_OPT_ADAM)) finish_dm(c);
    if (P.pre && P.pre_cached) {
        if (P.build_wT) launch_transpose_w(c->params + c->table_floats, c->L, c->wT, c->stream);
    } else if (P.pre) {
        if (int rc = grow_pass_buffer(c, P.pre_n + 16)) return rc;
        PassPrepArgs pa;
        memset(&pa, 0, sizeof(pa));
        pa.user_tab = c->user_tab;
        pa.item_tab = c->item_tab;
        pa.uid = d->uid;
        pa.pid = d->pid;
        pa.dom = d->dom;
        pa.label = d->label;
        pa.perm = d_perm;
        pa.pos0 = P.pre_pos0;
        pa.n = P.pre_n;
        pa.n_rows_split = d->n;
        pa.n_user = c->cfg.n_user;
        pa.n_item = c->cfg.n_item;
        pa.n_domain = c->cfg.n_domain;
        pa.pad_dom = domain;
        pa.xpre = c->xpre;
        pa.pdom = c->pdom;
        pa.plabel = c->plabel;
        if (P.build_wT) {
            pa.tw_dense = c->params + c->table_floats;
            pa.tw_L = c->L;
            pa.tw_wT = c->wT;
        }
        Prof p(c, MAMDR_KERNEL_AUX);
        launch_pass_prep(pa, c->stream);
    } else if (P.build_wT) {
        launch_transpose_w(c->params + c->table_floats, c->L, c->wT, c->stream);
    }
    if (optimizer != MAMDR_OPT_ACCUMULATE) c->wT_valid = P.need_wT;
    else if (P.build_wT) c->wT_valid = true;
    for (int64_t s = 0; s < n_steps; ++s) {
        if (d_loss_out) sync_tables(c);
        const float alpha = advance_step(c, optimizer, lr);
// ... 212 lines not shown
    if (n_seg < 0 || n_seg > PCG_MAX_SEG) return fail(MAMDR_EINVAL, "n_seg %d outside [0, %d]", n_seg, PCG_MAX_SEG);
    PcgArgs a;
    memset(&a, 0, sizeof(a));
    a.fin = d_final;
    a.aux = d_aux;
    a.n_seg = n_seg;
    for (int i = 0; i < n_seg; ++i) {
        if (h_offsets[i] < 0 || h_rows[i] < 0 || h_cols[i] <= 0 || h_cols[i] > 4096)
            return fail(MAMDR_EINVAL, "tensor %d: bad offset / rows / cols", i);
        a.off[i] = h_offsets[i];
        a.cols[i] = h_cols[i];
        a.row_start[i + 1] = a.row_start[i] + h_rows[i];
    }
    launch_pcgrad(a, (hipStream_t)stream);
    HIP_TRY(hipGetLastError());
    return MAMDR_OK;
}
int mamdr_copy(float* d_dst, const float* d_src, int64_t n, void* stream) {
    if (!d_dst || !d_src) return fail(MAMDR_EINVAL, "null pointer");
    if (n < 0) return fail(MAMDR_EINVAL, "negative length");
    if (n == 0) return MAMDR_OK;
    if (n == 0) return MAMDR_OK;
    HIP_TRY(hipMemcpyAsync(d_dst, d_src, (size_t)n * sizeof(float), hipMemcpyDeviceToDevice, (hipStream_t)stream));
    return MAMDR_OK;
}

int mamdr_shuffle_perm(int64_t n, int64_t buffer_size, uint64_t seed, int32_t* h_out) {
    if (n < 0 || n > 0x7fffffff) return fail(MAMDR_EINVAL, "n out of range");
    if (n == 0) return MAMDR_OK;
    if (!h_out) return fail(MAMDR_EINVAL, "null output");
    if (buffer_size < 1) buffer_size = 1;
    int64_t filled = n < buffer_size ? n : buffer_size;
    std::vector<int32_t> buf((size_t)filled);
    for (int64_t i = 0; i < filled; ++i) buf[(size_t)i] = (int32_t)i;
    int64_t next = filled;
    uint64_t state = seed;
    for (int64_t i = 0; i < n; ++i) {
        state += 0x9E3779B97F4A7C15ull;
        uint64_t z = state;
        z = (z ^ (z >> 30)) * 0xBF58476D1CE4E5B9ull;
        z = (z ^ (z >> 27)) * 0x94D049BB133111EBull;
        z = z ^ (z >> 31);
        const uint64_t j = ((z >> 32) * (uint64_t)filled) >> 32;
        h_out[i] = buf[(size_t)j];
        if (next < n) {
            buf[(size_t)j] = (int32_t)next++;
        } else {
            buf[(size_t)j] = buf[(size_t)filled - 1];
            --filled;
        }
    }
    return MAMDR_OK;
}

int mamdr_shuffle_perms(int32_t n_passes, const int64_t* h_n, int64_t buffer_size, const uint64_t* h_seeds,
                        int32_t* h_out) {
    if (n_passes < 0 || (n_passes > 0 && (!h_n || !h_seeds))) return fail(MAMDR_EINVAL, "bad pass list");
    int64_t off = 0;
    for (int32_t k = 0; k < n_passes; ++k) {
        const int rc = mamdr_shuffle_perm(h_n[k], buffer_size, h_seeds[k], h_out ? h_out + off : nullptr);
        if (rc) return rc;
        off += h_n[k];
    }
    return MAMDR_OK;
}

#ifdef MAMDR_STAMPS
int mamdr_debug_set_stamps(mamdr_ctx* c, unsigned long long* d_stamps) {
    c->stamps = d_stamps;
    return MAMDR_OK;
}
#endif

int64_t mamdr_dropout_steps(const mamdr_ctx* c) { return c ? (int64_t)c->global_step : 0; }

int mamdr_step_path(const mamdr_ctx* c, int32_t batch) { return c && takes_fused_path(c, batch) ? 1 : 0; }

int mamdr_set_tower_tile(mamdr_ctx* c, int32_t rows) {
    if (check_ctx(c)) return MAMDR_EINVAL;
    if (rows != 0 && rows != 4 && rows != 16) return fail(MAMDR_EINVAL, "tower tile of %d rows (0 = automatic, 4, 16)", rows);
    if (rows == 16 && (c->pnn || c->nfm)) return fail(MAMDR_EINVAL, "the pnn / nfm towers exist as four-row tiles only");
    if (rows != c->tower_tile) {
        c->tower_tile = rows;
        c->pg.clear();
        c->w1t_unread = w1t_unread_now(c);
        c->wT_valid = false;
    }
    return MAMDR_OK;
}
int mamdr_tower_tile(const mamdr_ctx* c, int32_t batch) {
    if (!c || batch <= 0) return MAMDR_EINVAL;
    return takes_tower4(c, pad_rows(batch)) ? 4 : 16;
}
int mamdr_profile_enable(mamdr_ctx* c, int32_t enable) {
    if (check_ctx(c)) return MAMDR_EINVAL;
    c->profile = enable != 0;
    return MAMDR_OK;
}
int mamdr_profile_reset(mamdr_ctx* c) {
    if (check_ctx(c)) return MAMDR_EINVAL;
    HIP_TRY(hipStreamSynchronize(c->stream));
    for (int k = 0; k < MAMDR_KERNEL_COUNT; ++k) {
        for (EventPair& p : c->ev[k]) {
            if (p.own_a) c->ev_pool_push(p.a);
            c->ev_pool_push(p.b);
        }
        c->ev[k].clear();
    }
    c->prev_b = nullptr;
    c->chain_ok = false;
    return MAMDR_OK;
}
int mamdr_profile_read(mamdr_ctx* c, int32_t kernel, double* total_ms, int64_t* launches) {
    if (check_ctx(c)) return MAMDR_EINVAL;
    if (kernel < 0 || kernel >= MAMDR_KERNEL_COUNT || !total_ms || !launches) return fail(MAMDR_EINVAL, "bad argument");
    HIP_TRY(hipStreamSynchronize(c->stream));
    double sum = 0.0;
    for (EventPair& p : c->ev[kernel]) {
        float ms = 0.f;
        HIP_TRY(hipEventElapsedTime(&ms, p.a, p.b));
        sum += ms;
    }
    *total_ms = sum;
    *launches = (int64_t)c->ev[kernel].size();
    return MAMDR_OK;
}

}
```

mamdr_amd/csrc/mamdr_kernels.h:

```cpp
#pragma once
#include <hip/hip_runtime.h>
#include <hip/hip_ext.h>
#include <stdint.h>

#include "mamdr_device.h"

namespace mamdr {

struct OptArgsLite {
    int optimizer;
    float alpha;
    float omb1, omb2, eps;
    float two_l2;
};
constexpr int32_t EMB_UNTOUCHED = 0x7fffffff;

extern thread_local hipEvent_t g_prof_stop;
int env_warn_unknown();
#define MAMDR_LAUNCH(kernel, grid, block, lds, stream, ...)                                               \
    do {                                                                                                  \
        if (::mamdr::g_prof_stop) {                                                                       \
            hipExtLaunchKernelGGL(kernel, grid, block, lds, stream, nullptr, ::mamdr::g_prof_stop, 0, __VA_ARGS__); \
            ::mamdr::g_prof_stop = nullptr;                                                               \
        } else {                                                                                          \
            hipLaunchKernelGGL(kernel, grid, block, lds, stream, __VA_ARGS__);                            \
        }                                                                                                 \
    } while (0)

constexpr int DM_PARTS = 32;
constexpr int DM_PAIRS = DM_PARTS / 2;
struct DmStep {
    const float* snap;
    const float* pdm;
    int n_part, n_domain;
    int optimizer;
    float alpha, omb1, omb2, eps, two_l2;
};
__device__ __forceinline__ f32x4 dm_pair(const DmStep& q, int d, int c4, int j) {
#pragma clang fp contract(off)
    const size_t row = (size_t)d * EMB + 4 * c4, plane = (size_t)q.n_domain * EMB;
    const f32x4 a = *reinterpret_cast<const f32x4*>(q.pdm + (size_t)(2 * j) * plane + row);
    const f32x4 b = *reinterpret_cast<const f32x4*>(q.pdm + (size_t)(2 * j + 1) * plane + row);
    return a + b;
}
__device__ __forceinline__ void dm_load4(const DmStep& q, int d, int c4, f32x4& p, f32x4& m, f32x4& v) {
    const size_t row = (size_t)d * EMB + 4 * c4, plane = (size_t)q.n_domain * EMB;
    p = *reinterpret_cast<const f32x4*>(q.snap + row);
    m = *reinterpret_cast<const f32x4*>(q.snap + plane + row);
    v = *reinterpret_cast<const f32x4*>(q.snap + 2 * plane + row);
}
__device__ __forceinline__ void dm_apply4(const DmStep& q, f32x4 g, f32x4& p, f32x4& m, f32x4& v) {
#pragma clang fp contract(off)
#pragma unroll
    for (int k = 0; k < 4; ++k) {
        const float gk = g[k] + q.two_l2 * p[k];
        if (q.optimizer == 0) {
            m[k] = m[k] + (gk - m[k]) * q.omb1;
            v[k] = v[k] + (gk * gk - v[k]) * q.omb2;
            p[k] = p[k] - (m[k] * q.alpha) / (sqrtf(v[k]) + q.eps);
        } else if (q.optimizer == 1) {
            p[k] = p[k] - gk * q.alpha;
        } else {
            m[k] = m[k] + gk;
        }
    }
}
__device__ __forceinline__ void dm_step4(const DmStep& q, int d, int c4, f32x4& p, f32x4& m, f32x4& v) {
#pragma clang fp contract(off)
    static_assert(DM_PAIRS == 16, "four groups of four pair sums");
    dm_load4(q, d, c4, p, m, v);
    f32x4 G[4];
#pragma unroll
    for (int gq = 0; gq < 4; ++gq) {
        f32x4 t[4];
#pragma unroll
        for (int k = 0; k < 4; ++k) t[k] = dm_pair(q, d, c4, 4 * gq + k);
        G[gq] = ((t[0] + t[1]) + t[2]) + t[3];
    }
    const f32x4 g = ((G[0] + G[1]) + G[2]) + G[3];
    dm_apply4(q, g, p, m, v);
}

struct TowerArgs {
    const float* user_tab;
    const float* item_tab;
    const float* dense;
    DenseLayout L;
    int n_user, n_item, n_domain;
// ... 223 lines not shown
        dm_pair_load(a.dms, d_read, c4, grp + 8, t.pr[1]);
        if (wr) {
            dm_pair_load(a.dms, dw, c4, grp, t.pw[0]);
            dm_pair_load(a.dms, dw, c4, grp + 8, t.pw[1]);
        }
    }
    const size_t plane = (size_t)a.n_domain * EMB;
    const int c = lp & (EMB - 1);
    if (wv < 6) {
        if (pend) {
            const size_t e = (size_t)d_read * EMB + c;
            t.p = a.dms.snap[e];
            t.m = a.dms.snap[plane + e];
            t.v = a.dms.snap[2 * plane + e];
        }
    } else if (wr) {
        const size_t e = (size_t)dw * EMB + c;
        if (pend) {
            t.p = a.dms.snap[e];
            t.m = a.dms.snap[plane + e];
            t.v = a.dms.snap[2 * plane + e];
        } else {
            t.p = a.dm_live_p[e];
            t.m = a.dm_live_m[e];
            t.v = a.dm_live_v[e];
        }
    }
}
__device__ __forceinline__ void dm_tile_stage(const TowerArgs& a, int tile, const DmTile& t, float* parts) {
    if (!a.dms.snap || threadIdx.x < 256) return;
    const int lp = (int)threadIdx.x - 256;
    *reinterpret_cast<f32x4*>(parts + lp * 4) = dm_pair_add(t.pr[0]);
    *reinterpret_cast<f32x4*>(parts + 1024 + lp * 4) = dm_pair_add(t.pr[1]);
    if (tile < a.n_domain) {
        *reinterpret_cast<f32x4*>(parts + 2048 + lp * 4) = dm_pair_add(t.pw[0]);
        *reinterpret_cast<f32x4*>(parts + 3072 + lp * 4) = dm_pair_add(t.pw[1]);
    }
}
__device__ __forceinline__ float dm_tile_reader(const TowerArgs& a, int c, const float* parts, const DmTile& t) {
    float p = t.p, m = t.m, v = t.v;
    dm_elem_finish(a.dms, c, parts, p, m, v);
    return p;
}
__device__ __forceinline__ void dm_store_elem(const TowerArgs& a, size_t e, bool stepped, float p, float m, float v) {
    const size_t plane = (size_t)a.n_domain * EMB;
    if (stepped) {
        if (a.dms.optimizer != 2) a.dm_live_p[e] = p;
        if (a.dms.optimizer != 1) a.dm_live_m[e] = m;
        if (a.dms.optimizer == 0) a.dm_live_v[e] = v;
    }
    a.dm_snap_out[e] = p;
    a.dm_snap_out[plane + e] = m;
    a.dm_snap_out[2 * plane + e] = v;
}
__device__ __forceinline__ void dm_tile_writer(const TowerArgs& a, int tile, int n_tiles, int c, const float* parts,
                                               const DmTile& t) {
    const bool pend = a.dms.snap != nullptr;
    if (tile < a.n_domain) {
        float p = t.p, m = t.m, v = t.v;
        if (pend) dm_elem_finish(a.dms, c, parts + 2048, p, m, v);
        dm_store_elem(a, (size_t)tile * EMB + c, pend, p, m, v);
    }
    if (c < EMB / 4) {
        for (int d = tile + n_tiles; d < a.n_domain; d += n_tiles) {
            f32x4 p, m, v;
            const size_t row = (size_t)d * EMB + 4 * c, plane = (size_t)a.n_domain * EMB;
            if (pend) {
                dm_step4(a.dms, d, c, p, m, v);
                if (a.dms.optimizer != 2) *reinterpret_cast<f32x4*>(a.dm_live_p + row) = p;
                if (a.dms.optimizer != 1) *reinterpret_cast<f32x4*>(a.dm_live_m + row) = m;
                if (a.dms.optimizer == 0) *reinterpret_cast<f32x4*>(a.dm_live_v + row) = v;
            } else {
                p = *reinterpret_cast<const f32x4*>(a.dm_live_p + row);
                m = *reinterpret_cast<const f32x4*>(a.dm_live_m + row);
                v = *reinterpret_cast<const f32x4*>(a.dm_live_v + row);
            }
            *reinterpret_cast<f32x4*>(a.dm_snap_out + row) = p;
            *reinterpret_cast<f32x4*>(a.dm_snap_out + plane + row) = m;
            *reinterpret_cast<f32x4*>(a.dm_snap_out + 2 * plane + row) = v;
        }
    }
}

struct FusedArgs {
    const float* acts;
    const float* dz;
    const float* dlogit;
    const int32_t* domrow;
    const float* xa;
    int xa_ld;
    int rows_pad, rows;
    float* p;
    float* m;
    float* v;
    DenseLayout L;
    int n_domain;
    const float* dm_snap;
    float* pdm;
    float* wT;
    int w1t_unread;
    int optimizer;
    float alpha, omb1, omb2, eps, two_l2;
    const float* loss_part;
    int n_loss_tiles;
    const float* frozen_sumsq;
    float l2_emb;
    float* loss_out;
#ifdef MAMDR_STAMPS
    unsigned long long* stamps;
#endif
};
void launch_wgrad_adam(const FusedArgs& a, hipStream_t s);
struct PassPrepArgs {
    const float* user_tab;
    const float* item_tab;
    const int32_t* uid;
    const int32_t* pid;
    const int32_t* dom;
    const float* label;
    const int32_t* perm;
    int64_t pos0, n, n_rows_split;
    int n_user, n_item, n_domain;
    int pad_dom;
    float* xpre;
    int32_t* pdom;
    float* plabel;
    const float* tw_dense;
    DenseLayout tw_L;
    float* tw_wT;
    int n_prep_wgs;
};
constexpr int PREP_MAX_PASSES = 16;
struct PassPrepMultiArgs {
    const float* user_tab;
    const float* item_tab;
    int n_user, n_item, n_domain, n_pass;
    float* xpre;
    int32_t* pdom;
    float* plabel;
    int wg_end[PREP_MAX_PASSES];
    struct Pass {
        const int32_t* uid;
        const int32_t* pid;
        const int32_t* dom;
        const float* label;
        const int32_t* perm;
        int64_t n, n_rows_split, out_off;
        int pad_dom;
    } p[PREP_MAX_PASSES];
};
void launch_pass_prep_multi(const PassPrepMultiArgs& a, hipStream_t s);
template <int ROWS>
__device__ __forceinline__ void w1_image_request(const float* __restrict__ W1, float* w1s, const int row0) {
    const int lane = threadIdx.x & 63;
    const uint32_t base = __builtin_amdgcn_readfirstlane((uint32_t)(uintptr_t)(w1s + row0 * H2));
#pragma unroll
    for (int kk = 0; kk < ROWS; kk += 2) {
        const int k = row0 + kk + (lane >> 5);
        const float* src = W1 + k * H2 + 4 * ((lane & 31) ^ (k & 31));
        const uint32_t dst = base + kk * H2 * 4;
        unsigned keep;
        asm volatile("s_mov_b32 %0, m0\n\ts_mov_b32 m0, %2\n\ts_nop 0\n\tglobal_load_lds_dwordx4 %1, off\n\ts_mov_b32 m0, %0"
                     : "=&s"(keep) : "v"(src), "s"(dst) : "memory");
    }
}
__device__ __forceinline__ void w1_image_landed() { asm volatile("s_waitcnt vmcnt(0)" ::: "memory"); }
__device__ __forceinline__ int w1_image_at(int row, int chunk) { return row * H2 + 4 * (chunk ^ (row & 31)); }

constexpr int TRANSPOSE_WGS = (WT_FLOATS + 255) / 256;
__device__ __forceinline__ void transpose_w_elem(const float* dense, const DenseLayout& L, float* wT, int e) {
    if (e < H1 * H2) {
        const int r = e / H2, c = e - r * H2;
        wT[W1T_OFF + c * H1 + r] = dense[L.w1 + e];
    } else if (e < H1 * H2 + H2 * H3) {
        const int f = e - H1 * H2;
        const int r = f / H3, c = f - r * H3;
        wT[W2T_OFF + c * H2 + r] = dense[L.w2 + f];
    } else if (e < WT_FLOATS) {
        const int f = e - (H1 * H2 + H2 * H3);
        const int r = f / H1, c = f - r * H1;
        wT[W0T_OFF + c * (2 * EMB) + r] = dense[L.w0 + f];
    }
}
void launch_pass_prep(const PassPrepArgs& a, hipStream_t s);
void launch_dm_finish(const DmStep& q, float* live_p, float* live_m, float* live_v, hipStream_t s);

void launch_tower_train(const TowerArgs& a, hipStream_t s);
void launch_tower_eval(const TowerArgs& a, hipStream_t s);
constexpr int T4_E_W2D_LDS = 1;
constexpr int T4_E_W2D_STATE = 2;
int launch_tower4_train(const TowerArgs& a, hipStream_t s);
bool tower4_w1l_ready();
bool tower4_takes_w1l(int64_t rows, int no_w1l);
bool tower4_never_streams(int64_t max_rows, int no_w1l);
void launch_transpose_w(const float* dense, const DenseLayout& L, float* wT, hipStream_t s);
struct EvalFinishArgs {
    const float* loss_part;
    int64_t n_rows;
    int batch;
    const float* dense;
    int dm_count;
    float l2_emb;
    const float* frozen_sumsq;
    int ld_off, ld_count;
    float l2_lin;
    float* loss_out;
};
void launch_eval_finish(const EvalFinishArgs& a, hipStream_t s);
struct GatherPf;
void launch_wgrad(const WgradArgs& a, hipStream_t s, const GatherPf* pf = nullptr);
struct GatherPf {
    const int32_t *perm, *uid, *pid, *dom;
    const float* label;
    const float *user_tab, *item_tab;
    int64_t row_base, n_rows_split;
    int rows, n_user, n_item, n_tiles;
    float* sink;
};
void launch_update(const UpdateArgs& a, hipStream_t s);
void launch_gather(const TowerArgs& a, float* out, hipStream_t s);
void launch_sumsq(const float* x, int64_t n, float* partials , float* out, hipStream_t s);

size_t tower_lds_bytes();

struct EmbTable {
    int64_t n_rows;
    const int32_t* brow;
    int32_t* map;
    float* gbuf;
    int32_t* hasdup;
// ... 146 lines not shown
```

mamdr_amd/engine.py:

```python
import ctypes as C

import numpy as np
import torch

from . import _lib as L


def _ptr(t):
    return C.c_void_p(t.data_ptr()) if t is not None else C.c_void_p(0)


def auc_thresholds(num_thresholds=500):
    inner = [(i + 1) * 1.0 / (num_thresholds - 1) for i in range(num_thresholds - 2)]
    return np.array([0.0 - 1e-7] + inner + [1.0 + 1e-7], dtype=np.float32)


def auc_from_histogram(hist):
    hist = np.asarray(hist, dtype=np.int64).reshape(2, 501)
    suffix = np.cumsum(hist[:, ::-1], axis=1)[:, ::-1]
    tp = suffix[1, 1:].astype(np.float32)
    fp = suffix[0, 1:].astype(np.float32)
    fn = (hist[1].sum() - suffix[1, 1:]).astype(np.float32)
    tn = (hist[0].sum() - suffix[0, 1:]).astype(np.float32)

# ... 366 lines not shown

    @property
    def adam_v(self):
        self.sync()
        return self._adam_v

    def keras_key(self):
        return self.tower, None, ()

    def pack(self, named):
        if "W0x" in self.segments and "W0x" not in named:
            w0 = np.asarray(named["W0"], np.float32).reshape(-1, 256)
            named = dict(named, W0=w0[:384], W0x=w0[384:])
        return DeviceEngine.pack(self, named)

    def unpack(self, vec):
        out = DeviceEngine.unpack(self, vec)
        if "W0x" in out:
            out["W0"] = np.concatenate([out["W0"], out.pop("W0x")])
        return out

    def set_weights(self, vec):
        dst = self.meta_weights if (self.meta_off and vec.numel() == self.n_meta) else self.weights
        L.check(self.lib.mamdr_copy(_ptr(dst), _ptr(vec), vec.numel(), self._s()))

    def get_weights(self, out=None):
        if out is None:
            out = torch.empty_like(self.weights)
        L.check(self.lib.mamdr_copy(_ptr(out), _ptr(self.weights), self.n_params, self._s()))
        return out

    def segment_shapes(self):
        D = self.n_domain
        out = {}
        for name, (off, cnt) in self.segments.items():
            if name in ("user_emb", "item_emb", "domain_emb"):
                out[name] = (cnt // 128, 128)
            elif name in ("W0", "Ws0"):
                out[name] = (cnt // 256, 256)
            elif name == "W0x":
                out[name] = (3, 256)
            elif name in ("W1", "Ws1"):
                out[name] = (256, 128)
            elif name in ("W2", "Ws2"):
                out[name] = (128, 64)
            elif name in ("Wd0", "Wd1", "Wd2"):
                cols = {"Wd0": 256, "Wd1": 128, "Wd2": 64}[name]
                out[name] = (cnt // cols, cols)
            elif name in ("bd0", "bd1", "bd2", "pn_gamma_spec", "pn_beta_spec"):
                out[name] = (D, cnt // D)
            elif name in ("wo", "lin_user", "lin_item", "lin_domain", "log_var", "gb"):
                out[name] = (cnt, 1)
            else:
                out[name] = (1, cnt)
        return out

    def set_tower_tile(self, rows):
        L.check(self.lib.mamdr_set_tower_tile(self.ctx, int(rows)))

    def tower_tile(self, batch=None):
        rows = int(self.lib.mamdr_tower_tile(self.ctx, int(batch or self.batch_size)))
        if rows < 0:
            L.check(rows)
        return rows

    def dr_advance(self, phi, merged, theta, gamma, method="plus", assign_model=True):
        mode = {"plus": L.MERGE_PLUS, "times": L.MERGE_TIMES}[method]
        holes = bool(self.meta_holes) and assign_model
        L.check(self.lib.mamdr_dr_advance_live(self.ctx, _ptr(phi), _ptr(merged), _ptr(theta), float(gamma), mode,
                                               1 if (assign_model and not holes) else 0, self.meta_off, phi.numel()))
        if holes:
            self.assign_meta(merged)

    def pregather(self, passes, batch_size=None):
        n = len(passes)
        if n == 0:
            L.check(self.lib.mamdr_pregather_passes(self.ctx, 0, None, None, None, int(batch_size or self.batch_size)))
            return
        doms = (C.c_int32 * n)(*[int(p[0]) for p in passes])
        perms = (C.c_void_p * n)(*[(p[1].data_ptr() if p[1] is not None else None) for p in passes])
        rows = (C.c_int64 * n)(*[(-1 if len(p) < 3 or p[2] is None else int(p[2])) for p in passes])
        L.check(self.lib.mamdr_pregather_passes(self.ctx, n, doms, perms, rows, int(batch_size or self.batch_size)))

    def gather(self, domain, split, perm=None, first_row=0, n_rows=None, out=None):
        n = self.n_rows(domain, split) if n_rows is None else n_rows
        if out is None:
            out = torch.empty((n, 384), dtype=torch.float32, device=self.device)
        split_id = {"train": L.SPLIT_TRAIN, "val": L.SPLIT_VAL, "test": L.SPLIT_TEST}[split]
        L.check(self.lib.mamdr_gather_rows(self.ctx, domain, split_id, _ptr(perm), first_row, n, _ptr(out)))
        return out

    def step_kernel_names(self, batch=None):
        fused = int(self.lib.mamdr_step_path(self.ctx, int(batch or self.batch_size))) == 1
        return {L.KERNEL_FWD_BWD: "k_tower<train>", L.KERNEL_WGRAD: "k_wgrad_adam" if fused else "k_wgrad",
                L.KERNEL_UPDATE: "k_dm_finish (when the live table is read)" if fused else "k_update"}

    def profile(self, enable):
        L.check(self.lib.mamdr_profile_enable(self.ctx, 1 if enable else 0))

    def profile_reset(self):
        L.check(self.lib.mamdr_profile_reset(self.ctx))

    def profile_read(self, kernel):
        ms, cnt = C.c_double(), C.c_int64()
        L.check(self.lib.mamdr_profile_read(self.ctx, kernel, C.byref(ms), C.byref(cnt)))
        return ms.value, cnt.value


def shuffle_perm(n, buffer_size, seed):
    out = np.empty(n, np.int32)
    L.check(L.load().mamdr_shuffle_perm(n, buffer_size, seed & 0xFFFFFFFFFFFFFFFF, out.ctypes.data))
    return out
```

mamdr_amd/meta.py:

```python
import torch


def _upload_perm(eng, perm):
    if perm is None:
        return None
    if isinstance(perm, torch.Tensor):
        return perm
    return torch.from_numpy(perm).to(eng.device, non_blocking=True)


class PassWindow(object):

    def __init__(self, eng, perm_fn, batch_size, budget_rows=96 * 1024, max_passes=16):
        self.eng, self.perm_fn, self.batch_size = eng, perm_fn, batch_size
        self.budget, self.max_passes = budget_rows, max_passes
        import os
        self.on = hasattr(perm_fn, "peek") and hasattr(eng, "pregather") and not os.environ.get("MAMDR_NO_PASS_WINDOW")
        if os.environ.get("MAMDR_PASS_WINDOW_ROWS"):
            self.budget = int(os.environ["MAMDR_PASS_WINDOW_ROWS"])
        self.todo, self.left = [], 0

    def announce(self, domains):
        self.todo, self.left = list(domains), 0

    def step(self):
        if not self.on:
            return
        if self.left == 0 and self.todo:
            take, rows = 0, 0
            while take < len(self.todo) and take < self.max_passes:
                n = self.eng.n_rows(self.todo[take], "train")
                if take and rows + n > self.budget:
                    break
                rows += n
                take += 1
            chunk, self.todo = self.todo[:take], self.todo[take:]
            perms = self.perm_fn.peek(chunk)
            if perms is None:
                self.on = False
                return
            self.eng.pregather(list(zip(chunk, perms)) if take > 1 else [], self.batch_size)
            self.left = take
        self.left = max(self.left - 1, 0)


def run_pass(eng, d, perm_fn, batch_size, lr, trace, phase, max_steps=0, optimizer="adam", window=None):
    if window is None:
        perm = _upload_perm(eng, perm_fn(d) if perm_fn is not None else None)
        n, pass_rows = eng.n_rows(d, "train"), None
    else:
        import numpy as np
        perm = perm_fn(d, window) if perm_fn is not None else None
        if perm is None:
            perm = np.arange(window[0], window[1], dtype=np.int32)
        perm = _upload_perm(eng, perm)
        n = pass_rows = window[1] - window[0]
    n_steps = -(-n // batch_size)
    if max_steps and max_steps > 0:
        n_steps = min(n_steps, max_steps)
    if pass_rows is None:
        eng.train_steps(d, perm=perm, first_step=0, n_steps=n_steps, lr=lr, optimizer=optimizer,
                        batch_size=batch_size)
    else:
        eng.train_steps(d, perm=perm, first_step=0, n_steps=n_steps, lr=lr, optimizer=optimizer,
                        batch_size=batch_size, pass_rows=pass_rows)
    trace.append((phase, d, n_steps))
    return n_steps


def alternate_epoch(eng, seq, perm_fn, batch_size, lr):
    trace = []
    for d in seq:
        run_pass(eng, d, perm_fn, batch_size, lr, trace, "alt")
    return trace


def dn_epoch(eng, theta, seq, perm_fn, batch_size, lr, meta_lr, meta_train_step=0, target=-1):
    trace = []
    eng.assign_meta(theta)
    for d in seq:
        run_pass(eng, d, perm_fn, batch_size, lr, trace, "dn", meta_train_step)
    if target >= 0:
        run_pass(eng, target, perm_fn, batch_size, lr, trace, "dn")
    eng.interp(theta, eng.meta_weights, theta, meta_lr)
    eng.assign_meta(theta)
    if target >= 0:
        run_pass(eng, target, perm_fn, batch_size, lr, trace, "target")
    return trace


def reptile_epoch(eng, theta, seq, perm_fn, batch_size, lr, meta_lr, batch_variant=False, meta_train_step=0,
                  acc=None, target=-1):
    trace = []
    if batch_variant and acc is None:
        acc = torch.zeros_like(theta)
    for d in seq:
        if target >= 0 and d == target:
            continue
        eng.assign_meta(theta)
        run_pass(eng, d, perm_fn, batch_size, lr, trace, "reptile", meta_train_step)
        if target >= 0:
            run_pass(eng, target, perm_fn, batch_size, lr, trace, "target_step", 1)
        if batch_variant:
            eng.accumulate(acc, eng.meta_weights, theta)
        else:
            eng.interp(theta, eng.meta_weights, theta, meta_lr)
    if batch_variant:
        eng.apply_accumulated(theta, acc, 0.0, meta_lr)
    eng.assign_meta(theta)
    if target >= 0:
        run_pass(eng, target, perm_fn, batch_size, lr, trace, "target")
    return trace


class OuterAdamState(object):

    def __init__(self, eng):
        import numpy as np
        self.m = eng.new_vector()
        self.v = eng.new_vector()
        self.b1p = np.float32(1.0)
        self.b2p = np.float32(1.0)

    def apply(self, eng, theta, acc, lr, grad_scale=1.0, clear=True):
        import numpy as np
        self.b1p = np.float32(self.b1p * np.float32(0.9))
        self.b2p = np.float32(self.b2p * np.float32(0.999))
        n = theta.numel()
        off = getattr(eng, "meta_off", 0) if (n != acc.numel() or n != self.m.numel()) else 0
        g = acc if acc.numel() == n else acc[off:off + n]
        m = self.m if self.m.numel() == n else self.m[off:off + n]
        v = self.v if self.v.numel() == n else self.v[off:off + n]
        eng.adam_apply(theta, m, v, g, lr, float(self.b1p), float(self.b2p), grad_scale)
        if clear:
            acc.zero_()


def maml_epoch(eng, theta, outer, acc, seq, perm_fn, batch_size, lr, meta_lr, batch_variant=False,
               meta_train_step=0, grad_scale=1.0, windows=None, meta_domain=-1):
    trace = []
    for d in seq:
        wt, wm = windows[d] if windows else (None, None)
        dm = d
        if meta_domain >= 0:
            dm, wm = meta_domain, None
        eng.assign_meta(theta)
        run_pass(eng, d, perm_fn, batch_size, lr, trace, "maml_train", meta_train_step, window=wt)
        run_pass(eng, dm, perm_fn, batch_size, lr, trace, "maml_meta", meta_train_step, optimizer="accumulate",
                 window=wm)
        if not batch_variant:
            outer.apply(eng, theta, acc, meta_lr, grad_scale)
    if batch_variant:
        outer.apply(eng, theta, acc, meta_lr, grad_scale)
    eng.assign_meta(theta)
    return trace


def mldg_epoch(eng, theta, outer, acc, seq, perm_fn, batch_size, lr, meta_lr, batch_variant=False,
               meta_train_step=0, grad_scale=1.0, windows=None, meta_domain=-1):
    trace = []
    for d in seq:
        wt, wm = windows[d] if windows else (None, None)
        eng.assign_meta(theta)
        run_pass(eng, d, perm_fn, batch_size, lr, trace, "mldg_train", meta_train_step, optimizer="accumulate",
                 window=wt)
        live = eng.meta_weights.clone()
        outer.apply(eng, live, acc, meta_lr, grad_scale, clear=False)
        eng.assign_meta(live)
        dm = d
        if meta_domain >= 0:
            dm, wm = meta_domain, None
        run_pass(eng, dm, perm_fn, batch_size, lr, trace, "mldg_meta", meta_train_step, optimizer="accumulate",
                 window=wm)
        if not batch_variant:
            eng.assign_meta(theta)
            outer.apply(eng, theta, acc, meta_lr, grad_scale)
    if batch_variant:
        eng.assign_meta(theta)
        outer.apply(eng, theta, acc, meta_lr, grad_scale)
    eng.assign_meta(theta)
    return trace


def pcgrad_epoch(eng, outer, cur, aux, seq, aux_plan, perm_fn, batch_size, lr, meta_lr, meta_train_step=0,
                 grad_scale=1.0, windows=None):
    trace = []
    tensors = None
    if eng.n_meta != eng.n_params and hasattr(eng, "segment_shapes"):
        shapes = eng.segment_shapes()
        lo, hi = eng.meta_off, eng.meta_off + eng.n_meta
        tensors = [(off, shapes[n][0], shapes[n][1]) for n, (off, cnt) in eng.segments.items() if off >= lo and off + cnt <= hi]
    for d in seq:
        eng.bind_accumulator(cur)
        cur.zero_()
        run_pass(eng, d, perm_fn, batch_size, lr, trace, "pcgrad_query", meta_train_step, optimizer="accumulate",
                 window=windows[d][0] if windows else None)
        for a in aux_plan[d]:
            eng.bind_accumulator(aux)
            aux.zero_()
            run_pass(eng, a, perm_fn, batch_size, lr, trace, "pcgrad_aux", 0, optimizer="accumulate",
                     window=windows[a][0] if windows else None)
            eng.pcgrad_project(cur, aux, tensors)
        live = eng.meta_weights.clone()
        outer.apply(eng, live, cur, meta_lr, grad_scale)
        eng.assign_meta(live)
    return trace


def dr_query(eng, theta, phi, query, support, perm_fn, batch_size, lr, meta_lr, trace, merged,
             merged_method="plus", domain_regulation_step=0, batch_variant=False, sample_num=None, acc=None, pw=None):
    eng.merge(merged, theta, phi, merged_method)
    if batch_variant:
        acc.zero_()
    assigned = False
    if pw is None:
        pw = PassWindow(eng, perm_fn, batch_size)
    capped = bool(domain_regulation_step and domain_regulation_step > 0)
    pw.announce([] if capped else [x for j in support for x in (j, query)])
    for k, j in enumerate(support):
        if not assigned:
            eng.assign_meta(merged)
        pw.step()
        run_pass(eng, j, perm_fn, batch_size, lr, trace, "dr_support")
        pw.step()
        run_pass(eng, query, perm_fn, batch_size, lr, trace, "dr_query", domain_regulation_step)
        if batch_variant:
            shared = theta if merged_method == "times" else None
            eng.accumulate(acc, eng.meta_weights, merged, shared, 1.0)
        else:
            assigned = k + 1 < len(support)
            eng.dr_advance(phi, merged, theta, meta_lr, merged_method, assign_model=assigned)
    if batch_variant:
        eng.apply_accumulated(phi, acc, float(sample_num), meta_lr)


def finetune_query(eng, theta, phi, query, perm_fn, batch_size, lr, trace, merged, merged_method="plus"):
    eng.merge(merged, theta, phi, merged_method)
    eng.assign_meta(merged)
    run_pass(eng, query, perm_fn, batch_size, lr, trace, "dr_finetune")
    eng.sub(phi, eng.meta_weights, merged)


def mamdr_epoch(eng, theta, phis, plan, perm_fn, batch_size, lr, meta_lr, merged_method="plus",
                domain_regulation_step=0, batch_variant=False, sample_num=None, scratch=None,
                finetune_every_epoch=False):
    trace = []
    pw = PassWindow(eng, perm_fn, batch_size)
    eng.assign_meta(theta)
    pw.announce(plan["seq"])
    for d in plan["seq"]:
        pw.step()
        run_pass(eng, d, perm_fn, batch_size, lr, trace, "dn")
    eng.interp(theta, eng.meta_weights, theta, meta_lr)
    merged = scratch if scratch is not None else torch.empty_like(theta)
    acc = torch.zeros_like(theta) if batch_variant else None
    for query, support in plan["dr"]:
        dr_query(eng, theta, phis[query], query, support, perm_fn, batch_size, lr, meta_lr, trace, merged,
                 merged_method, domain_regulation_step, batch_variant, sample_num, acc, pw)
        if finetune_every_epoch:
            finetune_query(eng, theta, phis[query], query, perm_fn, batch_size, lr, trace, merged, merged_method)
    return trace
```

mamdr_amd/parallel.py:

```python
import threading

import torch
import torch.distributed as dist

_lane = threading.local()


class LaneGroup(object):

    def __init__(self, n, outer=None, sum_block=None):
        self.n = int(n)
        if outer is None:
            outer = (dist.get_rank(), dist.get_world_size()) if (dist.is_available() and dist.is_initialized()) else (0, 1)
        self.outer_rank, self.outer_ws = int(outer[0]), int(outer[1])
        self.sum_block = int(sum_block) if sum_block else self.n
        if self.n % self.sum_block:
            raise ValueError("sum_block %d does not divide %d lanes" % (self.sum_block, self.n))
        self.barrier = threading.Barrier(self.n)
        self.slots = [None] * self.n
        self.ev = [None] * self.n
        self.ev2 = [None] * self.n
        self.adders = [None] * self.n

    def run(self, fn):
# ... 555 lines not shown
        g = lanes()
        if g is not None and (g.outer_ws == 1 or (P2P_ENABLED and p2p_possible(self.pack.device))):
            g.transfer(_lane.rank, self.phis, moves)
            return sum(self.P * 4 for _, src, _ in moves if src == rank)
        p2p = g is None and P2P_ENABLED and p2p_possible(self.pack.device)
        if p2p:
            ops = []
            for d, src, dst in moves:
                if rank == src:
                    ops.append(dist.P2POp(dist.isend, self.phis[d], dst))
                    sent += self.P * 4
                elif rank == dst:
                    ops.append(dist.P2POp(dist.irecv, self.phis[d], src))
            if ops:
                for req in dist.batch_isend_irecv(ops):
                    req.wait()
        else:
            for d, src, dst in moves:
                broadcast(self.phis[d], src)
                sent += self.P * 4 if rank == src else 0
        return sent

    def sync_phis(self):
        rank, ws = world()
        if ws > 1:
            for d in self.domains:
                if self.where[d] is not None:
                    broadcast(self.phis[d], self.where[d])
        self.where = {d: None for d in self.domains}

    def sync_tail(self):
        self.tail.sync()

    def _assign(self, plan, domain_regulation_step=0):
        rank, ws = world()
        if self.dn_mode == "replicated":
            dr_owner, _, load = epoch_assignment({"seq": [], "dr": plan["dr"]}, self.steps, ws, domain_regulation_step)
            dn_owner = {d: rank for d in plan["seq"]}
            load = [l + sum(self.steps[d] for d in plan["seq"]) for l in load]
        else:
            dr_owner, dn_owner, load = epoch_assignment(plan, self.steps, ws, domain_regulation_step)
        local = {"seq": [d for d in plan["seq"] if dn_owner[d] == rank],
                 "dr": [(q, s) for (q, s) in plan["dr"] if dr_owner[q] == rank]}
        return dr_owner, dn_owner, load, local

    def local_passes(self, plan, domain_regulation_step=0):
        from . import plan as mplan
        rank, ws = world()
        if ws == 1:
            return mplan.epoch_passes(plan, domain_regulation_step)
        return mplan.epoch_passes(self._assign(plan, domain_regulation_step)[3], domain_regulation_step)

    def epoch(self, plan, perm_prepare, perm_fn, batch_size, lr, meta_lr, merged_method="plus",
              domain_regulation_step=0, batch_variant=False, sample_num=None, finetune_every_epoch=False):
        from . import plan as mplan
        rank, ws = world()
        eng, meta, theta = self.eng, self.meta, self.theta
        if perm_prepare is not None and finetune_every_epoch:
            raise ValueError("pre-drawn epoch shuffles do not cover the per-query finetune passes")
        import time
        t_host = time.perf_counter()
        if ws == 1:
            if perm_prepare is not None:
                perm_prepare(mplan.epoch_passes(plan, domain_regulation_step))
            self.host_prep_s += time.perf_counter() - t_host
            return meta.mamdr_epoch(eng, theta, self.phis, plan, perm_fn, batch_size, lr, meta_lr, merged_method,
                                    domain_regulation_step, batch_variant, sample_num, scratch=self.merged,
                                    finetune_every_epoch=finetune_every_epoch)
        replicated = self.dn_mode == "replicated"
        dr_owner, dn_owner, load, local = self._assign(plan, domain_regulation_step)
        self.last_load = load
        if perm_prepare is not None:
            perm_prepare(mplan.epoch_passes(local, domain_regulation_step))
        self.host_prep_s += time.perf_counter() - t_host
        wire = self._transfer([(q, self.where[q], dr_owner[q]) for q, _ in sorted(plan["dr"])
                               if self.where[q] is not None and self.where[q] != dr_owner[q]])
        trace = []
        acc = torch.zeros_like(theta) if batch_variant else None
        if replicated and self.tail.active:
            self.tail.sync()
            wire += self.tail.floats() * 4
        eng.assign_meta(theta)
        pw = meta.PassWindow(eng, perm_fn, batch_size)
        pw.announce(local["seq"])
        for d in local["seq"]:
            pw.step()
            meta.run_pass(eng, d, perm_fn, batch_size, lr, trace, "dn")
        if replicated:
            live = eng.weights
            if self.tail.active:
                broadcast(live, 0)
                if self.tail.aux is not None:
                    broadcast(self.tail.aux, 0)
                self.tail.rebase()
                wire += live.numel() * 4 if rank == 0 else 0
                eng.sub(self.delta, live[:self.P], theta)
            else:
                eng.sub(self.delta, live, theta)
                broadcast(self.delta, 0)
                wire += self.P * 4 if rank == 0 else 0
        else:
            eng.sub(self.delta, eng.meta_weights, theta)
            if self.tail.active:
                self.tail.fill(self.tail_buf)
                all_reduce(self.pack[:self.P + self.tail_buf.numel()])
                self.tail.apply(self.tail_buf)
                wire += (self.P + self.tail_buf.numel()) * 4
            else:
                all_reduce(self.delta)
                wire += self.P * 4
        eng.interp(theta, self.delta, self.zero, meta_lr)
        for query, support in local["dr"]:
            meta.dr_query(eng, theta, self.phis[query], query, support, perm_fn, batch_size, lr, meta_lr, trace,
                          self.merged, merged_method, domain_regulation_step, batch_variant, sample_num, acc)
            if finetune_every_epoch:
                meta.finetune_query(eng, theta, self.phis[query], query, perm_fn, batch_size, lr, trace, self.merged,
                                    merged_method)
        self.mine = set(q for q, _ in local["dr"])
        for q, _ in plan["dr"]:
            self.where[q] = dr_owner[q]
        self.wire_bytes.append(wire)
        return trace


def broadcast_live(eng, src=0):
    rank, ws = world()
    if ws <= 1:
        return
    w = eng.weights
    broadcast(w, src)
    if w.data_ptr() != eng.weights.data_ptr():
        eng.set_weights(w)
    aux = getattr(eng, "aux", None)
    if aux is not None:
        broadcast(aux, src)


def gather_domain_scalars(local, n_domain, device):
    rank, ws = world()
    t = torch.zeros(n_domain, 3, dtype=torch.float64, device=device)
    for d, (loss, auc) in local.items():
        t[d, 0], t[d, 1], t[d, 2] = loss, auc, 1.0
    if ws > 1:
        all_reduce(t)
    t = t.cpu()
    return ({d: float(t[d, 0]) for d in range(n_domain) if t[d, 2] > 0},
            {d: float(t[d, 1]) for d in range(n_domain) if t[d, 2] > 0})
```

Baseline: 45330 domain-steps/s.

## Pre-gather the next pass window using rider workgroups inside k_wgrad_adam

While the current pass window runs, the rows for the next window are gathered ahead of time. Extra 'rider' workgroups are appended to the fused k_wgrad_adam grid to fill CUs the kernel leaves idle, and they write embedding rows, domains and labels into a second set of buffers. The Python PassWindow now peeks at the permutations for the following chunk, including the DR-phase announcements, so the next window's k_pass_prep launch shrinks or disappears. The cost is a second set of pregather buffers, more complex bookkeeping, and riders that may contend with the weight-gradient and Adam work for memory bandwidth.

After: 45840 domain-steps/s (median of 6 runs). 1.01x the previous value.

```diff
diff --git a/include/mamdr_hip.h b/include/mamdr_hip.h
--- a/include/mamdr_hip.h
+++ b/include/mamdr_hip.h
@@ -136,8 +136,12 @@
 int mamdr_profile_enable(mamdr_ctx* ctx, int32_t enable);
 int mamdr_pregather_passes(mamdr_ctx* ctx, int32_t n_passes, const int32_t* h_domains, const int32_t* const* h_d_perms,
                            const int64_t* h_pass_rows, int32_t batch);
+int mamdr_pregather_ahead(mamdr_ctx* ctx, int32_t n_passes, const int32_t* h_domains, const int32_t* const* h_d_perms,
+                          const int64_t* h_pass_rows, int32_t batch, int64_t spread_steps);
 int64_t mamdr_pregather_hits(const mamdr_ctx* ctx);
 int64_t mamdr_pregather_launches(const mamdr_ctx* ctx);
+int64_t mamdr_pregather_rider_rows(const mamdr_ctx* ctx);
+int64_t mamdr_pregather_remainder_rows(const mamdr_ctx* ctx);
 int mamdr_step_path(const mamdr_ctx* ctx, int32_t batch);
 int mamdr_set_tower_tile(mamdr_ctx* ctx, int32_t rows);
 int mamdr_tower_tile(const mamdr_ctx* ctx, int32_t batch);
diff --git a/mamdr_amd/_lib.py b/mamdr_amd/_lib.py
--- a/mamdr_amd/_lib.py
+++ b/mamdr_amd/_lib.py
@@ -86,6 +86,9 @@
     "mamdr_pregather_passes": (_I32, [_VP, _I32, _VP, _VP, _VP, _I32]),
     "mamdr_pregather_hits": (_I64, [_VP]),
     "mamdr_pregather_launches": (_I64, [_VP]),
+    "mamdr_pregather_ahead": (_I32, [_VP, _I32, _VP, _VP, _VP, _I32, _I64]),
+    "mamdr_pregather_rider_rows": (_I64, [_VP]),
+    "mamdr_pregather_remainder_rows": (_I64, [_VP]),
     "mamdr_sync_tables": (C.c_int, [_VP]),
     "mamdr_bind_accumulator": (C.c_int, [_VP, _VP]),
     "mamdr_bind_table": (C.c_int, [_VP, C.c_int, _VP, _I64]),
diff --git a/mamdr_amd/csrc/env_registry.h b/mamdr_amd/csrc/env_registry.h
--- a/mamdr_amd/csrc/env_registry.h
+++ b/mamdr_amd/csrc/env_registry.h
@@ -20,6 +20,7 @@
     {"MAMDR_T4_NO_W1L", "lib", "1: k_tower4 without the W1 image in LDS (diagnostic)"},
     {"MAMDR_NO_W2_DIRECT", "lib", "1: k_transpose_w opens a call instead of the W2-in-place tower instance"},
     {"MAMDR_NO_PREGATHER", "lib,bench", "1: no k_pass_prep; the tower gathers its rows itself"},
+    {"MAMDR_NO_PREGATHER_RIDE", "lib", "1: no rider workgroups in k_wgrad_adam; every pass window is gathered by k_pass_prep_multi (same bits)"},
     {"MAMDR_STAR_DENSE_SLICES", "lib", "1: every per-domain Star slice swept every step (diagnostic; same bits)"},
     {"MAMDR_GRAPH_NO_DEFER", "lib", "1: a pair of weight-gradient launches per layer instead of the queued flat grid"},
     {"MAMDR_GRAPH_TILE32_BELOW", "lib", "row count below which the 32 x 32 GEMM tile is used (0: 64 x 64 everywhere)"},
diff --git a/mamdr_amd/csrc/fused_kernels.hip b/mamdr_amd/csrc/fused_kernels.hip
--- a/mamdr_amd/csrc/fused_kernels.hip
+++ b/mamdr_amd/csrc/fused_kernels.hip
@@ -14,6 +14,7 @@
 constexpr int FZ_T1 = (H1 / 16) * (H2 / 32);
 constexpr int FZ_T2 = (H2 / 16) * (H3 / 32);
 constexpr int FZ_TILES = FZ_T0 + FZ_T1 + FZ_T2;
+__host__ __device__ constexpr int fz_own_wgs(bool with_loss) { return FZ_SBLK + FZ_TILES + FZ_OUTB + (with_loss ? 1 : 0); }
 
 #define FZSTAMP(k) MAMDR_STAMP(MAMDR_CYCLES, a.stamps && threadIdx.x == 0, a.stamps[blockIdx.x * 8 + (k)])
 #define FZREAL(k) MAMDR_STAMP(MAMDR_REALTIME, a.stamps && threadIdx.x == 0, a.stamps[blockIdx.x * 8 + (k)])
@@ -458,6 +459,90 @@
     }
 }
 
+template <typename P>
+__device__ __forceinline__ void prep_ids(const P& a, int n_user, int n_item, int64_t pos, int64_t& src, int& u, int& it) {
+    src = a.perm ? (int64_t)a.perm[pos] : pos;
+    src = src < 0 ? 0 : (src >= a.n_rows_split ? a.n_rows_split - 1 : src);
+    u = a.uid[src];
+    it = a.pid[src];
+    u = u < 0 ? 0 : (u >= n_user ? n_user - 1 : u);
+    it = it < 0 ? 0 : (it >= n_item ? n_item - 1 : it);
+}
+__device__ __forceinline__ const f32x4* prep_src(const float* user_tab, const float* item_tab, int u, int it, int lane) {
+    return reinterpret_cast<const f32x4*>(lane < 32 ? user_tab + (size_t)u * EMB + 4 * lane : item_tab + (size_t)it * EMB + 4 * (lane - 32));
+}
+__device__ __forceinline__ void prep_store_row(float* xpre, int64_t i, int lane, f32x4 v) {
+    __builtin_nontemporal_store(v, reinterpret_cast<f32x4*>(xpre + (size_t)i * (2 * EMB) + 4 * lane));
+}
+template <typename P>
+__device__ __forceinline__ void prep_meta(const P& a, int n_domain, int64_t src, int32_t* pdom, float* plabel, int64_t i) {
+    const int d = a.dom[src];
+    pdom[i] = d < 0 ? 0 : (d >= n_domain ? n_domain - 1 : d);
+    plabel[i] = a.label[src];
+}
+__device__ __forceinline__ void prep_pad_row(float* xpre, int64_t i, int lane) {
+    *reinterpret_cast<f32x4*>(xpre + (size_t)i * (2 * EMB) + 4 * lane) = (f32x4){0.f, 0.f, 0.f, 0.f};
+}
+template <typename P>
+__device__ __forceinline__ void prep_pad_meta(const P& a, int32_t* pdom, float* plabel, int64_t i) {
+    pdom[i] = a.pad_dom;
+    plabel[i] = 0.f;
+}
+
+__device__ __forceinline__ int64_t ride_row(const RideArgs& g, int q) {
+    if (q < g.seg[0].count) return g.seg[0].out_off + g.seg[0].first + q;
+    q -= g.seg[0].count;
+    if (q < g.seg[1].count) return g.seg[1].out_off + g.seg[1].first + q;
+    return -1;
+}
+__device__ __forceinline__ void ride_resolve(const RideArgs& g, const RideArgs::Seg& s, int n_domain, int q, int& u, int& it) {
+    const int64_t i = (int64_t)s.first + q;
+    if (i < s.n) {
+        int64_t src;
+        prep_ids(s, g.n_user, g.n_item, i, src, u, it);
+        prep_meta(s, n_domain, src, g.pdom + s.out_off, g.plabel + s.out_off, i);
+    } else {
+        prep_pad_meta(s, g.pdom + s.out_off, g.plabel + s.out_off, i);
+        u = -1;
+        it = 0;
+    }
+}
+__device__ __forceinline__ void fz_ride_body(const FusedArgs& a, int r, float* lds) {
+    const RideArgs& g = a.ride;
+    const int tid = threadIdx.x, lane = tid & 63;
+    const int w = __builtin_amdgcn_readfirstlane(tid >> 6);
+    int* ids = reinterpret_cast<int*>(lds);
+    if (tid < FZ_RIDE_ROWS) {
+        const int q = r * FZ_RIDE_ROWS + tid;
+        int u = -1, it = 0;
+        if (q < g.seg[0].count) ride_resolve(g, g.seg[0], a.n_domain, q, u, it);
+        else if (q - g.seg[0].count < g.seg[1].count) ride_resolve(g, g.seg[1], a.n_domain, q - g.seg[0].count, u, it);
+        *reinterpret_cast<int2*>(ids + 2 * tid) = make_int2(u, it);
+    }
+    FZSTAMP(1);
+    FZSTAMP(2);
+    __syncthreads();
+    FZSTAMP(3);
+    constexpr int PER = FZ_RIDE_ROWS / FZ_WAVES;
+    f32x4 v[PER];
+    int us[PER];
+#pragma unroll
+    for (int k = 0; k < PER; ++k) {
+        const int2 id = *reinterpret_cast<const int2*>(ids + 2 * (w * PER + k));
+        us[k] = __builtin_amdgcn_readfirstlane(id.x);
+        const int it = __builtin_amdgcn_readfirstlane(id.y);
+        v[k] = *prep_src(g.user_tab, g.item_tab, max(us[k], 0), it, lane);
+    }
+#pragma unroll
+    for (int k = 0; k < PER; ++k) {
+        const int64_t row = ride_row(g, r * FZ_RIDE_ROWS + w * PER + k);
+        if (row < 0) continue;
+        if (us[k] >= 0) prep_store_row(g.xpre, row, lane, v[k]);
+        else prep_pad_row(g.xpre, row, lane);
+    }
+    FZSTAMP(4);
+}
+
 __global__ __launch_bounds__(FZ_THREADS) void k_wgrad_adam(const FusedArgs a) {
     extern __shared__ __attribute__((aligned(16))) float lds[];
     const int b = (int)blockIdx.x;
@@ -466,12 +551,15 @@
     if (b < FZ_SBLK) fz_s_body(a, b, lds);
     else if (b < FZ_SBLK + FZ_TILES) fz_tile_body(a, b - FZ_SBLK, lds);
     else if (b < FZ_SBLK + FZ_TILES + FZ_OUTB) fz_out_body(a, b - FZ_SBLK - FZ_TILES, lds);
-    else fz_loss_body(a, lds);
+    else if (b < fz_own_wgs(a.loss_out != nullptr)) fz_loss_body(a, lds);
+    else fz_ride_body(a, b - fz_own_wgs(a.loss_out != nullptr), lds);
     FZREAL(6);
 }
 
+int wgrad_adam_own_wgs(bool with_loss) { return fz_own_wgs(with_loss); }
+
 void launch_wgrad_adam(const FusedArgs& a, hipStream_t s) {
-    const int grid = FZ_SBLK + FZ_TILES + FZ_OUTB + (a.loss_out ? 1 : 0);
+    const int grid = fz_own_wgs(a.loss_out != nullptr) + a.ride.n_wg;
     const size_t lds = (size_t)fz_lds_floats(a.n_domain) * sizeof(float);
     if (lds > 65536) {
         static const bool big_lds_set = hipFuncSetAttribute(reinterpret_cast<const void*>(k_wgrad_adam),
@@ -503,28 +591,18 @@
                                               int n_domain, int64_t pos0, float* xpre, int32_t* pdom, float* plabel, int64_t i) {
     const int lane = threadIdx.x & 63;
     if (i >= a.n) {
-        if (i < a.n + 16) {
-            *reinterpret_cast<f32x4*>(xpre + (size_t)i * (2 * EMB) + 4 * lane) = (f32x4){0.f, 0.f, 0.f, 0.f};
-            if (lane == 0) {
-                pdom[i] = a.pad_dom;
-                plabel[i] = 0.f;
-            }
+        if (i < a.n + PREP_PAD) {
+            prep_pad_row(xpre, i, lane);
+            if (lane == 0) prep_pad_meta(a, pdom, plabel, i);
         }
         return;
     }
-    int64_t src = a.perm ? (int64_t)a.perm[pos0 + i] : pos0 + i;
-    src = src < 0 ? 0 : (src >= a.n_rows_split ? a.n_rows_split - 1 : src);
-    int u = a.uid[src], it = a.pid[src];
-    u = u < 0 ? 0 : (u >= n_user ? n_user - 1 : u);
-    it = it < 0 ? 0 : (it >= n_item ? n_item - 1 : it);
-    const float* row = lane < 32 ? user_tab + (size_t)u * EMB + 4 * lane : item_tab + (size_t)it * EMB + 4 * (lane - 32);
-    const f32x4 v = *reinterpret_cast<const f32x4*>(row);
-    __builtin_nontemporal_store(v, reinterpret_cast<f32x4*>(xpre + (size_t)i * (2 * EMB) + 4 * lane));
-    if (lane == 0) {
-        int d = a.dom[src];
-        pdom[i] = d < 0 ? 0 : (d >= n_domain ? n_domain - 1 : d);
-        plabel[i] = a.label[src];
-    }
+    int64_t src;
+    int u, it;
+    prep_ids(a, n_user, n_item, pos0 + i, src, u, it);
+    const f32x4 v = *prep_src(user_tab, item_tab, u, it, lane);
+    prep_store_row(xpre, i, lane, v);
+    if (lane == 0) prep_meta(a, n_domain, src, pdom, plabel, i);
 }
 __global__ __launch_bounds__(256) void k_pass_prep(const PassPrepArgs a) {
     if ((int)blockIdx.x >= a.n_prep_wgs) {
@@ -540,7 +618,7 @@
     const int wg0 = k ? a.wg_end[k - 1] : 0;
     const PassPrepMultiArgs::Pass& p = a.p[k];
     pass_prep_row(p, a.user_tab, a.item_tab, a.n_user, a.n_item, a.n_domain, (int64_t)0, a.xpre + (size_t)p.out_off * (2 * EMB),
-                  a.pdom + p.out_off, a.plabel + p.out_off, (int64_t)((int)blockIdx.x - wg0) * 4 + (threadIdx.x >> 6));
+                  a.pdom + p.out_off, a.plabel + p.out_off, p.i0 + (int64_t)((int)blockIdx.x - wg0) * 4 + (threadIdx.x >> 6));
 }
 void launch_pass_prep_multi(const PassPrepMultiArgs& a, hipStream_t s) {
     if (a.n_pass <= 0) return;
diff --git a/mamdr_amd/csrc/mamdr_api.hip b/mamdr_amd/csrc/mamdr_api.hip
--- a/mamdr_amd/csrc/mamdr_api.hip
+++ b/mamdr_amd/csrc/mamdr_api.hip
@@ -110,6 +110,21 @@
     size_t pg_pos = 0;
     int64_t pg_hits = 0;
     int64_t pg_launches = 0;
+    float* xpre_ahead = nullptr;
+    int32_t* pdom_ahead = nullptr;
+    float* plabel_ahead = nullptr;
+    int64_t pre_cap_ahead = 0;
+    struct Ahead {
+        bool on = false;
+        std::vector<PgEntry> list;
+        std::vector<int64_t> rows;
+        PassPrepMultiArgs args;
+        PrePlanCursor cur;
+    } ahead;
+    int n_cu = 0;
+    bool ride_on = true;
+    int64_t pg_rider_rows = 0;
+    int64_t pg_remainder_rows = 0;
     bool use_pre = true;
     float* dmsnap[2] = {nullptr, nullptr};
     int dm_cur = 0;
@@ -445,6 +460,13 @@
 static int64_t pad_rows(int64_t rows) { return (rows + TILE_ROWS - 1) / TILE_ROWS * TILE_ROWS; }
 static int rows_at(int64_t pass_rows, int64_t row_base, int batch) { return (int)std::min<int64_t>(batch, pass_rows - row_base); }
 static bool takes_fused_path(const mamdr_ctx* c, int64_t batch) { return c->fused && pad_rows(batch) <= c->fused_max_batch; }
+static void drop_pregathered(mamdr_ctx* c) {
+    c->pg.clear();
+    c->ahead.on = false;
+}
+static int ride_wgs(const mamdr_ctx* c, bool with_loss) {
+    return std::max(0, std::min(FZ_RIDE_CAP, c->n_cu - wgrad_adam_own_wgs(with_loss)));
+}
 static bool takes_tower4(const mamdr_ctx* c, int64_t rows_pad) {
     return !c->star && c->tower_tile != 16 && (c->tower_tile == 4 || rows_pad <= c->tower4_max_rows);
 }
@@ -525,7 +547,7 @@
                 break;
             }
         }
-        if (!P.pre_cached) c->pg.clear();
+        if (!P.pre_cached) drop_pregathered(c);
     }
     P.star_lazy = c->star && P.optimizer == MAMDR_OPT_ADAM && P.n_steps >= 2 && !P.loss_out && !c->star_dense_slices &&
                   c->cfg.n_domain > 1;
@@ -793,6 +815,39 @@
     return MAMDR_OK;
 }
 
+static void attach_riders(mamdr_ctx* c, FusedArgs& fa) {
+    mamdr_ctx::Ahead& h = c->ahead;
+    const int riders = ride_wgs(c, fa.loss_out != nullptr);
+    if (riders <= 0) return;
+    const PrePlanSlice sl = pre_plan_next(h.rows.data(), (int)h.rows.size(), h.cur, (int64_t)riders * FZ_RIDE_ROWS);
+    if (sl.count() <= 0) return;
+    RideArgs& g = fa.ride;
+    g.user_tab = c->user_tab;
+    g.item_tab = c->item_tab;
+    g.xpre = c->xpre_ahead;
+    g.pdom = c->pdom_ahead;
+    g.plabel = c->plabel_ahead;
+    g.n_user = c->cfg.n_user;
+    g.n_item = c->cfg.n_item;
+    g.n_wg = (int)((sl.count() + FZ_RIDE_ROWS - 1) / FZ_RIDE_ROWS);
+    for (int k = 0; k < sl.n_seg; ++k) {
+        const PassPrepMultiArgs::Pass& p = h.args.p[sl.seg[k].pass];
+        RideArgs::Seg& q = g.seg[k];
+        q.uid = p.uid;
+        q.pid = p.pid;
+        q.dom = p.dom;
+        q.label = p.label;
+        q.perm = p.perm;
+        q.out_off = p.out_off;
+        q.n = (int)p.n;
+        q.n_rows_split = (int)p.n_rows_split;
+        q.first = (int)sl.seg[k].first;
+        q.count = (int)sl.seg[k].count;
+        q.pad_dom = p.pad_dom;
+    }
+    c->pg_rider_rows += sl.count();
+}
+
 static int fused_step(mamdr_ctx* c, const CallPlan& P, int64_t s, float alpha) {
     const int32_t optimizer = P.optimizer;
     const int64_t row_base = (P.first_step + s) * P.batch;
@@ -851,6 +906,7 @@
 #ifdef MAMDR_STAMPS
     fa.stamps = c->stamps ? c->stamps + 65536 + (c->global_step & 1) * 4096 : nullptr;
 #endif
+    if (c->ahead.on && !c->profile) attach_riders(c, fa);
     {
         Prof p(c, MAMDR_KERNEL_WGRAD);
         launch_wgrad_adam(fa, c->stream);
@@ -1185,6 +1241,7 @@
             if (hipGetDevice(&dev) != hipSuccess || hipDeviceGetAttribute(&n_cu, hipDeviceAttributeMultiprocessorCount, dev) != hipSuccess ||
                 n_cu <= 0)
                 n_cu = 256;
+            c->n_cu = n_cu;
             const int one_round = std::min(2048, std::max(256, 4 * n_cu));
             c->fused_max_batch = one_round;
             if (cfg->tower == MAMDR_TOWER_MLP && !cfg->emb_trainable) c->tower4_max_rows = one_round;
@@ -1201,6 +1258,7 @@
             if (const char* de = getenv("MAMDR_DM_CALL")) c->dm_finish_call = atoi(de) != 0;
             if (const char* de = getenv("MAMDR_NO_W2_DIRECT")) c->w2_direct_ok = atoi(de) == 0;
             if (const char* pe = getenv("MAMDR_NO_PREGATHER")) c->use_pre = atoi(pe) == 0;
+            if (const char* pe = getenv("MAMDR_NO_PREGATHER_RIDE")) c->ride_on = atoi(pe) == 0;
         }
         c->w1t_unread = w1t_unread_now(c);
     }
@@ -1243,7 +1301,7 @@
             (void)hipEventDestroy(p.b);
         }
     for (hipEvent_t e : c->ev_pool) (void)hipEventDestroy(e);
-    void* ptrs[] = {c->urow_alt, c->irow_alt, c->map_u_alt, c->map_i_alt, c->acts, c->dz, c->dlogit, c->w0dom_copy, c->dm_copy, c->wT, c->dxe, c->urow, c->irow, c->map_u, c->map_i, c->gbuf_u, c->gbuf_i, c->hasdup_u, c->hasdup_i, c->last_u, c->last_i, c->alpha_log, c->star_alpha, c->pdm, c->dmsnap[0], c->dmsnap[1], c->xpre, c->pdom, c->plabel, c->fmq, c->ipbuf, c->glin_u, c->glin_i, c->eff, c->pn, c->star_part, c->star_sums, c->star_dmpart, c->domrow, c->loss_part, c->eval_part, c->slabs,
+    void* ptrs[] = {c->urow_alt, c->irow_alt, c->map_u_alt, c->map_i_alt, c->acts, c->dz, c->dlogit, c->w0dom_copy, c->dm_copy, c->wT, c->dxe, c->urow, c->irow, c->map_u, c->map_i, c->gbuf_u, c->gbuf_i, c->hasdup_u, c->hasdup_i, c->last_u, c->last_i, c->alpha_log, c->star_alpha, c->pdm, c->dmsnap[0], c->dmsnap[1], c->xpre, c->pdom, c->plabel, c->xpre_ahead, c->pdom_ahead, c->plabel_ahead, c->fmq, c->ipbuf, c->glin_u, c->glin_i, c->eff, c->pn, c->star_part, c->star_sums, c->star_dmpart, c->domrow, c->loss_part, c->eval_part, c->slabs,
                     c->tiles, c->thresholds, c->frozen_sumsq, c->sumsq_partials};
     for (void* p : ptrs)
         if (p) (void)hipFree(p);
@@ -1419,7 +1477,7 @@
     if (check_ctx(c)) return MAMDR_EINVAL;
     if (c->cfg.emb_trainable) return fail(MAMDR_ESTATE, "tables are trainable: they live in the flat vector");
     if (!d_rows || ((uintptr_t)d_rows & 15)) return fail(MAMDR_EINVAL, "table pointer null or not 16-byte aligned");
-    c->pg.clear();
+    drop_pregathered(c);
     if (seg == MAMDR_SEG_USER_EMB) {
         if (n_rows != c->cfg.n_user) return fail(MAMDR_EINVAL, "user table has %lld rows, config says %d", (long long)n_rows, c->cfg.n_user);
         c->user_tab = d_rows;
@@ -1448,7 +1506,7 @@
     d->dom = d_domain;
     d->label = d_label;
     d->n = n_rows;
-    c->pg.clear();
+    drop_pregathered(c);
     const int64_t tiles = (n_rows + TILE_ROWS - 1) / TILE_ROWS;
     if (tiles > c->eval_part_cap) {
         HIP_TRY(hipStreamSynchronize(c->stream));
@@ -1460,34 +1518,33 @@
     return MAMDR_OK;
 }
 
+static int grow_pass_set(float*& xpre, int32_t*& pdom, float*& plabel, int64_t& have, int64_t rows) {
+    if (rows <= have) return MAMDR_OK;
+    const int64_t cap = rows + rows / 4 + 1024;
+    if (xpre) { (void)hipFree(xpre); (void)hipFree(pdom); (void)hipFree(plabel); }
+    xpre = nullptr; pdom = nullptr; plabel = nullptr; have = 0;
+    HIP_TRY(hipMalloc((void**)&xpre, (size_t)cap * 2 * EMB * sizeof(float)));
+    HIP_TRY(hipMalloc((void**)&pdom, (size_t)cap * sizeof(int32_t)));
+    HIP_TRY(hipMalloc((void**)&plabel, (size_t)cap * sizeof(float)));
+    have = cap;
+    return MAMDR_OK;
+}
 static int grow_pass_buffer(mamdr_ctx* c, int64_t rows) {
     if (rows <= c->pre_cap) return MAMDR_OK;
-    const int64_t cap = rows + rows / 4 + 1024;
-    c->pg.clear();
-    if (c->xpre) { (void)hipFree(c->xpre); (void)hipFree(c->pdom); (void)hipFree(c->plabel); }
-    c->xpre = nullptr; c->pdom = nullptr; c->plabel = nullptr; c->pre_cap = 0;
-    HIP_TRY(hipMalloc((void**)&c->xpre, (size_t)cap * 2 * EMB * sizeof(float)));
-    HIP_TRY(hipMalloc((void**)&c->pdom, (size_t)cap * sizeof(int32_t)));
-    HIP_TRY(hipMalloc((void**)&c->plabel, (size_t)cap * sizeof(float)));
-    c->pre_cap = cap;
-    return MAMDR_OK;
+    drop_pregathered(c);
+    return grow_pass_set(c->xpre, c->pdom, c->plabel, c->pre_cap, rows);
 }
 
 int64_t mamdr_pregather_hits(const mamdr_ctx* c) { return c ? c->pg_hits : 0; }
 int64_t mamdr_pregather_launches(const mamdr_ctx* c) { return c ? c->pg_launches : 0; }
-
-int mamdr_pregather_passes(mamdr_ctx* c, int32_t n_passes, const int32_t* h_domains, const int32_t* const* h_d_perms,
-                           const int64_t* h_pass_rows, int32_t batch) {
-    if (check_ctx(c)) return MAMDR_EINVAL;
-    if (ready(c)) return MAMDR_ESTATE;
-    if (n_passes < 0 || (n_passes > 0 && !h_domains)) return fail(MAMDR_EINVAL, "pregather: bad pass list");
-    c->pg.clear();
-    c->pg_pos = 0;
-    if (n_passes == 0 || batch <= 0 || batch > c->cfg.max_batch || !c->use_pre || !takes_fused_path(c, batch))
-        return MAMDR_OK;
-    if (n_passes > PREP_MAX_PASSES) n_passes = PREP_MAX_PASSES;
-    PassPrepMultiArgs a;
+int64_t mamdr_pregather_rider_rows(const mamdr_ctx* c) { return c ? c->pg_rider_rows : 0; }
+int64_t mamdr_pregather_remainder_rows(const mamdr_ctx* c) { return c ? c->pg_remainder_rows : 0; }
+
+static int lay_out_passes(mamdr_ctx* c, int32_t n_passes, const int32_t* h_domains, const int32_t* const* h_d_perms,
+                          const int64_t* h_pass_rows, int32_t batch, PassPrepMultiArgs& a, std::vector<mamdr_ctx::PgEntry>& list,
+                          int64_t& total) {
     memset(&a, 0, sizeof(a));
+    list.clear();
     int64_t off = 0;
     int wgs = 0;
     for (int k = 0; k < n_passes; ++k) {
@@ -1507,34 +1564,101 @@
         p.n_rows_split = d->n;
         p.out_off = off;
         p.pad_dom = h_domains[k];
-        const int64_t w = n > 0 ? (n + 16 + 3) / 4 : 0;
+        const int64_t w = n > 0 ? (n + PREP_PAD + 3) / 4 : 0;
         wgs += (int)w;
         a.wg_end[k] = wgs;
-        c->pg.push_back(mamdr_ctx::PgEntry{h_domains[k], p.perm, n, off, batch});
+        list.push_back(mamdr_ctx::PgEntry{h_domains[k], p.perm, n, off, batch});
         off += 4 * w;
     }
     a.n_pass = n_passes;
-    if (wgs == 0) return MAMDR_OK;
-    {
-        std::vector<mamdr_ctx::PgEntry> keep = c->pg;
-        if (int rc = grow_pass_buffer(c, off)) return rc;
-        c->pg = keep;
-    }
     a.user_tab = c->user_tab;
     a.item_tab = c->item_tab;
     a.n_user = c->cfg.n_user;
     a.n_item = c->cfg.n_item;
     a.n_domain = c->cfg.n_domain;
+    total = off;
+    return MAMDR_OK;
+}
+static bool pregather_applies(const mamdr_ctx* c, int32_t n_passes, int32_t batch) {
+    return n_passes > 0 && batch > 0 && batch <= c->cfg.max_batch && c->use_pre && takes_fused_path(c, batch);
+}
+
+int mamdr_pregather_passes(mamdr_ctx* c, int32_t n_passes, const int32_t* h_domains, const int32_t* const* h_d_perms,
+                           const int64_t* h_pass_rows, int32_t batch) {
+    if (check_ctx(c)) return MAMDR_EINVAL;
+    if (ready(c)) return MAMDR_ESTATE;
+    if (n_passes < 0 || (n_passes > 0 && !h_domains)) return fail(MAMDR_EINVAL, "pregather: bad pass list");
+    const bool had_ahead = c->ahead.on;
+    drop_pregathered(c);
+    c->pg_pos = 0;
+    if (!pregather_applies(c, n_passes, batch)) return MAMDR_OK;
+    if (n_passes > PREP_MAX_PASSES) n_passes = PREP_MAX_PASSES;
+    PassPrepMultiArgs a;
+    std::vector<mamdr_ctx::PgEntry> list;
+    int64_t total = 0;
+    if (int rc = lay_out_passes(c, n_passes, h_domains, h_d_perms, h_pass_rows, batch, a, list, total)) return rc;
+    if (total == 0) {
+        c->pg = list;
+        return MAMDR_OK;
+    }
+    mamdr_ctx::Ahead& h = c->ahead;
+    bool adopt = had_ahead && h.list.size() == list.size();
+    for (size_t k = 0; adopt && k < list.size(); ++k)
+        adopt = h.list[k].domain == list[k].domain && h.list[k].perm == list[k].perm && h.list[k].n == list[k].n &&
+                h.list[k].batch == list[k].batch;
+    if (adopt) {
+        std::swap(c->xpre, c->xpre_ahead);
+        std::swap(c->pdom, c->pdom_ahead);
+        std::swap(c->plabel, c->plabel_ahead);
+        std::swap(c->pre_cap, c->pre_cap_ahead);
+        pre_plan_settle(h.rows.data(), n_passes, h.cur);
+        int wgs = 0;
+        int64_t left = 0;
+        for (int k = 0; k < n_passes; ++k) {
+            const int64_t from = k < h.cur.pass ? pre_plan_positions(h.rows[k]) : (k == h.cur.pass ? h.cur.pos : 0);
+            const int64_t todo = pre_plan_positions(h.rows[k]) - from;
+            a.p[k].i0 = from;
+            wgs += (int)((todo + 3) / 4);
+            a.wg_end[k] = wgs;
+            left += todo;
+        }
+        if (left == 0) a.n_pass = 0;
+        c->pg_remainder_rows += left;
+    } else if (int rc = grow_pass_buffer(c, total)) {
+        return rc;
+    }
+    c->pg = list;
     a.xpre = c->xpre;
     a.pdom = c->pdom;
     a.plabel = c->plabel;
-    prof_break(c);
-    {
+    c->pg_launches++;
+    if (a.n_pass > 0) {
+        prof_break(c);
         Prof p(c, MAMDR_KERNEL_AUX);
         launch_pass_prep_multi(a, c->stream);
-        c->pg_launches++;
     }
     HIP_TRY(hipGetLastError());
+    return MAMDR_OK;
+}
+
+int mamdr_pregather_ahead(mamdr_ctx* c, int32_t n_passes, const int32_t* h_domains, const int32_t* const* h_d_perms,
+                          const int64_t* h_pass_rows, int32_t batch, int64_t spread_steps) {
+    if (check_ctx(c)) return MAMDR_EINVAL;
+    if (ready(c)) return MAMDR_ESTATE;
+    if (n_passes < 0 || (n_passes > 0 && !h_domains)) return fail(MAMDR_EINVAL, "pregather: bad pass list");
+    mamdr_ctx::Ahead& h = c->ahead;
+    h.on = false;
+    if (!pregather_applies(c, n_passes, batch) || spread_steps <= 0 || !c->ride_on || c->profile || ride_wgs(c, false) <= 0)
+        return MAMDR_OK;
+    if (n_passes > PREP_MAX_PASSES) n_passes = PREP_MAX_PASSES;
+    int64_t total = 0;
+    if (int rc = lay_out_passes(c, n_passes, h_domains, h_d_perms, h_pass_rows, batch, h.args, h.list, total)) return rc;
+    if (total == 0) return MAMDR_OK;
+    if (int rc = grow_pass_set(c->xpre_ahead, c->pdom_ahead, c->plabel_ahead, c->pre_cap_ahead, total)) return rc;
+    h.rows.clear();
+    for (const mamdr_ctx::PgEntry& e : h.list) h.rows.push_back(e.n);
+    h.cur = PrePlanCursor();
+    h.on = true;
     return MAMDR_OK;
 }
 
@@ -1913,7 +2037,7 @@
     if (rows == 16 && (c->pnn || c->nfm)) return fail(MAMDR_EINVAL, "the pnn / nfm towers exist as four-row tiles only");
     if (rows != c->tower_tile) {
         c->tower_tile = rows;
-        c->pg.clear();
+        drop_pregathered(c);
         c->w1t_unread = w1t_unread_now(c);
         c->wT_valid = false;
     }
diff --git a/mamdr_amd/csrc/mamdr_kernels.h b/mamdr_amd/csrc/mamdr_kernels.h
--- a/mamdr_amd/csrc/mamdr_kernels.h
+++ b/mamdr_amd/csrc/mamdr_kernels.h
@@ -4,6 +4,7 @@
 #include <stdint.h>
 
 #include "mamdr_device.h"
+#include "pregather_plan.h"
 
 namespace mamdr {
 
@@ -393,6 +394,26 @@
     }
 }
 
+constexpr int FZ_RIDE_ROWS = 64;
+constexpr int FZ_RIDE_CAP = 32;
+struct RideArgs {
+    const float* user_tab;
+    const float* item_tab;
+    float* xpre;
+    int32_t* pdom;
+    float* plabel;
+    int n_user, n_item;
+    int n_wg;
+    struct Seg {
+        const int32_t* uid;
+        const int32_t* pid;
+        const int32_t* dom;
+        const float* label;
+        const int32_t* perm;
+        int64_t out_off;
+        int n, n_rows_split, first, count, pad_dom;
+    } seg[2];
+};
 struct FusedArgs {
     const float* acts;
     const float* dz;
@@ -417,11 +438,13 @@
     const float* frozen_sumsq;
     float l2_emb;
     float* loss_out;
+    RideArgs ride;
 #ifdef MAMDR_STAMPS
     unsigned long long* stamps;
 #endif
 };
 void launch_wgrad_adam(const FusedArgs& a, hipStream_t s);
+int wgrad_adam_own_wgs(bool with_loss);
 struct PassPrepArgs {
     const float* user_tab;
     const float* item_tab;
@@ -457,6 +480,7 @@
         const float* label;
         const int32_t* perm;
         int64_t n, n_rows_split, out_off;
+        int64_t i0;
         int pad_dom;
     } p[PREP_MAX_PASSES];
 };
diff --git a/mamdr_amd/csrc/pregather_plan.h b/mamdr_amd/csrc/pregather_plan.h
--- /dev/null
+++ b/mamdr_amd/csrc/pregather_plan.h
@@ -0,0 +1,49 @@
+#pragma once
+
+#include <cstdint>
+
+namespace mamdr {
+
+constexpr int PREP_PAD = 16;
+
+struct PrePlanCursor {
+    int pass = 0;
+    int64_t pos = 0;
+};
+struct PrePlanSeg {
+    int pass = 0;
+    int64_t first = 0, count = 0;
+};
+struct PrePlanSlice {
+    int n_seg = 0;
+    PrePlanSeg seg[2];
+    int64_t count() const { return seg[0].count + seg[1].count; }
+};
+
+inline int64_t pre_plan_positions(int64_t rows) { return rows > 0 ? rows + PREP_PAD : 0; }
+
+inline void pre_plan_settle(const int64_t* pass_rows, int n_pass, PrePlanCursor& cur) {
+    while (cur.pass < n_pass && cur.pos >= pre_plan_positions(pass_rows[cur.pass])) {
+        cur.pass += 1;
+        cur.pos = 0;
+    }
+}
+
+inline PrePlanSlice pre_plan_next(const int64_t* pass_rows, int n_pass, PrePlanCursor& cur, int64_t quota) {
+    PrePlanSlice s;
+    while (s.n_seg < 2 && quota > 0) {
+        pre_plan_settle(pass_rows, n_pass, cur);
+        if (cur.pass >= n_pass) break;
+        const int64_t left = pre_plan_positions(pass_rows[cur.pass]) - cur.pos;
+        PrePlanSeg& g = s.seg[s.n_seg++];
+        g.pass = cur.pass;
+        g.first = cur.pos;
+        g.count = left < quota ? left : quota;
+        cur.pos += g.count;
+        quota -= g.count;
+    }
+    pre_plan_settle(pass_rows, n_pass, cur);
+    return s;
+}
+
+}
diff --git a/mamdr_amd/engine.py b/mamdr_amd/engine.py
--- a/mamdr_amd/engine.py
+++ b/mamdr_amd/engine.py
@@ -472,6 +472,14 @@
         rows = (C.c_int64 * n)(*[(-1 if len(p) < 3 or p[2] is None else int(p[2])) for p in passes])
         L.check(self.lib.mamdr_pregather_passes(self.ctx, n, doms, perms, rows, int(batch_size or self.batch_size)))
 
+    def pregather_ahead(self, passes, batch_size=None, spread_steps=0):
+        n = len(passes)
+        doms = (C.c_int32 * n)(*[int(p[0]) for p in passes])
+        perms = (C.c_void_p * n)(*[(p[1].data_ptr() if p[1] is not None else None) for p in passes])
+        rows = (C.c_int64 * n)(*[(-1 if len(p) < 3 or p[2] is None else int(p[2])) for p in passes])
+        L.check(self.lib.mamdr_pregather_ahead(self.ctx, n, doms, perms, rows, int(batch_size or self.batch_size),
+                                               int(spread_steps)))
+
     def gather(self, domain, split, perm=None, first_row=0, n_rows=None, out=None):
         n = self.n_rows(domain, split) if n_rows is None else n_rows
         if out is None:
diff --git a/mamdr_amd/meta.py b/mamdr_amd/meta.py
--- a/mamdr_amd/meta.py
+++ b/mamdr_amd/meta.py
@@ -18,30 +18,48 @@
         self.on = hasattr(perm_fn, "peek") and hasattr(eng, "pregather") and not os.environ.get("MAMDR_NO_PASS_WINDOW")
         if os.environ.get("MAMDR_PASS_WINDOW_ROWS"):
             self.budget = int(os.environ["MAMDR_PASS_WINDOW_ROWS"])
-        self.todo, self.left = [], 0
-
-    def announce(self, domains):
+        self.todo, self.left, self.then = [], 0, []
+
+    def announce(self, domains, then=()):
         self.todo, self.left = list(domains), 0
+        self.then = [list(g) for g in then]
+
+    def _cut(self, todo):
+        take, rows = 0, 0
+        while take < len(todo) and take < self.max_passes:
+            n = self.eng.n_rows(todo[take], "train")
+            if take and rows + n > self.budget:
+                break
+            rows += n
+            take += 1
+        return take
 
     def step(self):
         if not self.on:
             return
         if self.left == 0 and self.todo:
-            take, rows = 0, 0
-            while take < len(self.todo) and take < self.max_passes:
-                n = self.eng.n_rows(self.todo[take], "train")
-                if take and rows + n > self.budget:
-                    break
-                rows += n
-                take += 1
+            take = self._cut(self.todo)
             chunk, self.todo = self.todo[:take], self.todo[take:]
-            perms = self.perm_fn.peek(chunk)
+            after = next((g for g in [self.todo] + self.then if g), [])
+            after = after[:self._cut(after)]
+            ahead = hasattr(self.eng, "pregather_ahead") and take > 1 and len(after) > 1
+            perms = self.perm_fn.peek(chunk + after) if ahead else None
+            if perms is None:
+                ahead, perms = False, self.perm_fn.peek(chunk)
             if perms is None:
                 self.on = False
                 return
             self.eng.pregather(list(zip(chunk, perms)) if take > 1 else [], self.batch_size)
+            if ahead:
+                steps = sum(-(-self.eng.n_rows(d, "train") // self.batch_size) for d in chunk)
+                self.eng.pregather_ahead(list(zip(after, perms[take:])), self.batch_size, spread_steps=steps)
             self.left = take
         self.left = max(self.left - 1, 0)
+
+
+def dr_announcements(dr, domain_regulation_step=0):
+    capped = bool(domain_regulation_step and domain_regulation_step > 0)
+    return [[] if capped else [x for j in support for x in (j, query)] for query, support in dr]
 
 
 def run_pass(eng, d, perm_fn, batch_size, lr, trace, phase, max_steps=0, optimizer="adam", window=None):
@@ -208,15 +226,15 @@
 
 
 def dr_query(eng, theta, phi, query, support, perm_fn, batch_size, lr, meta_lr, trace, merged,
-             merged_method="plus", domain_regulation_step=0, batch_variant=False, sample_num=None, acc=None, pw=None):
+             merged_method="plus", domain_regulation_step=0, batch_variant=False, sample_num=None, acc=None, pw=None,
+             then=()):
     eng.merge(merged, theta, phi, merged_method)
     if batch_variant:
         acc.zero_()
     assigned = False
     if pw is None:
         pw = PassWindow(eng, perm_fn, batch_size)
-    capped = bool(domain_regulation_step and domain_regulation_step > 0)
-    pw.announce([] if capped else [x for j in support for x in (j, query)])
+    pw.announce(dr_announcements([(query, support)], domain_regulation_step)[0], then)
     for k, j in enumerate(support):
         if not assigned:
             eng.assign_meta(merged)
@@ -247,16 +265,17 @@
     trace = []
     pw = PassWindow(eng, perm_fn, batch_size)
     eng.assign_meta(theta)
-    pw.announce(plan["seq"])
+    later = [] if finetune_every_epoch else dr_announcements(plan["dr"], domain_regulation_step)
+    pw.announce(plan["seq"], later)
     for d in plan["seq"]:
         pw.step()
         run_pass(eng, d, perm_fn, batch_size, lr, trace, "dn")
     eng.interp(theta, eng.meta_weights, theta, meta_lr)
     merged = scratch if scratch is not None else torch.empty_like(theta)
     acc = torch.zeros_like(theta) if batch_variant else None
-    for query, support in plan["dr"]:
+    for k, (query, support) in enumerate(plan["dr"]):
         dr_query(eng, theta, phis[query], query, support, perm_fn, batch_size, lr, meta_lr, trace, merged,
-                 merged_method, domain_regulation_step, batch_variant, sample_num, acc, pw)
+                 merged_method, domain_regulation_step, batch_variant, sample_num, acc, pw, later[k + 1:])
         if finetune_every_epoch:
             finetune_query(eng, theta, phis[query], query, perm_fn, batch_size, lr, trace, merged, merged_method)
     return trace
diff --git a/mamdr_amd/parallel.py b/mamdr_amd/parallel.py
--- a/mamdr_amd/parallel.py
+++ b/mamdr_amd/parallel.py
@@ -661,7 +661,8 @@
             wire += self.tail.floats() * 4
         eng.assign_meta(theta)
         pw = meta.PassWindow(eng, perm_fn, batch_size)
-        pw.announce(local["seq"])
+        later = [] if finetune_every_epoch else meta.dr_announcements(local["dr"], domain_regulation_step)
+        pw.announce(local["seq"], later)
         for d in local["seq"]:
             pw.step()
             meta.run_pass(eng, d, perm_fn, batch_size, lr, trace, "dn")
@@ -689,9 +690,9 @@
                 all_reduce(self.delta)
                 wire += self.P * 4
         eng.interp(theta, self.delta, self.zero, meta_lr)
-        for query, support in local["dr"]:
+        for k, (query, support) in enumerate(local["dr"]):
             meta.dr_query(eng, theta, self.phis[query], query, support, perm_fn, batch_size, lr, meta_lr, trace,
-                          self.merged, merged_method, domain_regulation_step, batch_variant, sample_num, acc)
+                          self.merged, merged_method, domain_regulation_step, batch_variant, sample_num, acc, pw, later[k + 1:])
             if finetune_every_epoch:
                 meta.finetune_query(eng, theta, self.phis[query], query, perm_fn, batch_size, lr, trace, self.merged,
                                     merged_method)
```
